# marbl/Mash

Measured on AMD Instinct MI355X. Metric: pairwise Mash distances/sec (s=1000), higher is better.
Workload: dtype u64; 1 GPU; mash triangle all-vs-all, 100000 clustered synthetic sketches, k=21 s=1000, 4999950000 pairs/step, per-table job (index build + discover + fill + merge each step), row-block sharded x1; parallelism=rowblock1, rccl_ranks=0

## Files before the change

### mash_amd/csrc/compare_dense.hip

```cpp
#ifdef MG_HIP_EMU
#include "hipemu.h"
#else
#include <hip/hip_runtime.h>
#define MG_DYN_SHARED(T, name)                                   \
    extern __shared__ __align__(16) unsigned char name##_raw[]; \
    T *name = reinterpret_cast<T *>(name##_raw)
#endif
#include <stdint.h>

#include <cstdlib>

#ifndef MG_HIP_EMU
#include <rocprim/device/device_radix_sort.hpp>
#include <rocprim/device/device_select.hpp>
#include <rocprim/iterator/counting_iterator.hpp>
#endif

#include "compare_internal.h"

namespace mg {

#ifndef MG_HIP_EMU
__global__ __launch_bounds__(256) void dn_neighbor_kernel(const uint64_t *hashes, uint64_t stride, const uint32_t *cnt, uint32_t n,
                                                          uint8_t *link)
// ... 299 lines not shown
            }
            nx += total;
            __syncthreads();
        }
    }
    __syncthreads();
    const uint32_t jb = (row - G.g0) >> 7, bl = (row - G.g0) & 127u;
    const uint64_t bw = dense_block_words(W);
    unsigned long long *blk = gdata + G.data_off + (uint64_t)jb * bw;
    uint16_t *cxp = reinterpret_cast<uint16_t *>(blk + 128ull * W), *totp = cxp + (W + 1u) * 128u;
    unsigned long long *xpl = blk + dense_block_planes(W);
    for (uint32_t i = tid; i < 16u * W; i += 256u) {
        const uint32_t four = gap8[i], w = i >> 4, q = i & 15u;
        uint32_t bits[4] = {0u, 0u, 0u, 0u}, over = 0;
#pragma unroll
        for (uint32_t e = 0; e < 4u; e++) {
            const uint32_t c = (four >> (8u * e)) & 255u;
            over |= c >= 16u ? 1u : 0u;
#pragma unroll
            for (uint32_t j = 0; j < 4u; j++) bits[j] |= ((c >> j) & 1u) << ((4u * q + e) & 31u);
        }
        if (over || (q == 0 && hist[w] >= 256u)) ovf[w] = 1u;
#pragma unroll
        for (uint32_t j = 0; j < 4u; j++)
            if (bits[j]) atomicOr(&pl32[2u * (4u * w + j) + (q >> 3)], bits[j]);
    }
    __syncthreads();
    for (uint32_t i = tid; i < 4u * W; i += 256u) xpl[i * 128u + bl] = (unsigned long long)pl32[2u * i] | ((unsigned long long)pl32[2u * i + 1u] << 32);
    if (tid == 0) {
        uint32_t run = 0, all = 0;
        for (uint32_t w = 0; w <= W; w++) {
            cxp[w * 128u + bl] = (uint16_t)(run | ((w > 0 && ovf[w - 1u]) ? DN_CX_FLAG : 0u));
            totp[w * 128u + bl] = (uint16_t)all;
            if (w < W) {
                run += hist[w];
                all += hist[w] + (uint32_t)__popc(mask32[2u * w]) + (uint32_t)__popc(mask32[2u * w + 1u]);
            }
        }
    }
    for (uint32_t w = tid; w < W; w += 256u)
        blk[w * 128u + bl] = (unsigned long long)mask32[2u * w] | ((unsigned long long)mask32[2u * w + 1u] << 32);
}

hipError_t launch_dense_encode(const uint32_t *off, const uint32_t *code_img, uint32_t *pos_img, uint32_t rs, const uint32_t *grp_of,
                               const DenseGroup *groups, const uint32_t *ulist, const uint32_t *upos, unsigned long long *gdata,
                               uint16_t *ext, uint32_t xs, uint32_t n, uint32_t wmax, hipStream_t stream, int ul_mode)
{
    if (n == 0) return hipSuccess;
    const size_t fixed = ((size_t)28 * wmax + 9) * 4, with_ul = fixed + (size_t)wmax * 64 * 4;
    const bool ul_in_lds = ul_mode == 0 ? false : ul_mode == 1 ? with_ul <= 150 * 1024 : with_ul <= 40 * 1024;
    const size_t smem = ul_in_lds ? with_ul : fixed;
    auto go = [&](auto kern) -> hipError_t {
        hipError_t e = hipFuncSetAttribute(reinterpret_cast<const void *>(kern), hipFuncAttributeMaxDynamicSharedMemorySize, (int)smem);
        if (e != hipSuccess) return e;
        hipLaunchKernelGGL(kern, dim3((n + 63u) & ~63u), dim3(256), smem, stream, off, code_img, pos_img, rs, grp_of, groups, ulist, upos, gdata, wmax, ext, xs,
                           n, ul_in_lds ? 1u : 0u);
        return hipGetLastError();
    };
    return rs >= 4096u ? go(dn_encode_kernel<8>) : go(dn_encode_kernel<1>);
}



__device__ __forceinline__ uint32_t dn_count_add(uint32_t x, uint32_t acc)
{
#ifdef MG_HIP_EMU
    return (uint32_t)__popc(x) + acc;
#else
    uint32_t d;
    asm("v_bcnt_u32_b32 %0, %1, %2" : "=v"(d) : "v"(x), "v"(acc));
    return d;
#endif
}

__device__ __forceinline__ uint32_t dn_low_bits(uint32_t x, uint32_t y)
{
#ifdef MG_HIP_EMU
    return x & ((1u << y) - 1u);
#else
    return __builtin_amdgcn_ubfe(x, 0u, y);
#endif
}

template <uint32_t NP>
__device__ __forceinline__ uint32_t dn_descend(uint32_t base, uint32_t s, uint32_t u1, uint32_t A0, uint32_t B0, uint32_t A1, uint32_t B1,
                                               uint32_t A2, uint32_t B2, uint32_t A3, uint32_t B3)
{
    uint32_t pos = 0;
#pragma unroll
    for (uint32_t bit = 16u; bit != 0u; bit >>= 1) {
        const uint32_t y = pos + bit;
        uint32_t c = dn_count_add(dn_low_bits(B0, y), dn_count_add(dn_low_bits(A0, y), dn_count_add(dn_low_bits(u1, y), base)));
        if (NP >= 1u) c += 2u * dn_count_add(dn_low_bits(B1, y), (uint32_t)__popc(dn_low_bits(A1, y)));
        if (NP >= 3u)
            c += 4u * dn_count_add(dn_low_bits(B2, y), (uint32_t)__popc(dn_low_bits(A2, y))) +
                 8u * dn_count_add(dn_low_bits(B3, y), (uint32_t)__popc(dn_low_bits(A3, y)));
        pos = c < s ? y : pos;
    }
    return pos;
}

__device__ __forceinline__ uint32_t dn_resolve(unsigned long long un, unsigned long long mab, uint32_t fprev, uint32_t s, uint32_t w, bool lists,
                                               const unsigned long long *xpa, const unsigned long long *xpb, const uint16_t *xa,
                                               const uint16_t *xb, uint32_t ca0, uint32_t na, uint32_t cb0, uint32_t nb)
{
    if (__ballot(lists) == 0) {
        const unsigned long long a0 = xpa[512u * w], a1 = xpa[512u * w + 128u], a2 = xpa[512u * w + 256u], a3 = xpa[512u * w + 384u];
        const unsigned long long b0 = xpb[512u * w], b1 = xpb[512u * w + 128u], b2 = xpb[512u * w + 256u], b3 = xpb[512u * w + 384u];
        const bool p1 = __ballot((a1 | b1) != 0ull) != 0, p23 = __ballot((a2 | a3 | b2 | b3) != 0ull) != 0;
        const uint32_t ulo = (uint32_t)un, uhi = (uint32_t)(un >> 32);
        uint32_t c31 = dn_count_add((uint32_t)b0, dn_count_add((uint32_t)a0, dn_count_add(ulo & 0x7FFFFFFFu, fprev)));
        if (p1 || p23) c31 += 2u * dn_count_add((uint32_t)b1, (uint32_t)__popc((uint32_t)a1));
        if (p23)
            c31 += 4u * dn_count_add((uint32_t)b2, (uint32_t)__popc((uint32_t)a2)) + 8u * dn_count_add((uint32_t)b3, (uint32_t)__popc((uint32_t)a3));
        const bool upper = c31 < s;
        const uint32_t base = upper ? c31 + (ulo >> 31) : fprev;
        const uint32_t u1 = (upper ? uhi : ulo) << 1;
        const uint32_t A0 = upper ? (uint32_t)(a0 >> 32) : (uint32_t)a0, B0 = upper ? (uint32_t)(b0 >> 32) : (uint32_t)b0;
        uint32_t pos;
        if (!p1 && !p23) {
            pos = dn_descend<0>(base, s, u1, A0, B0, 0, 0, 0, 0, 0, 0);
        } else {
            const uint32_t A1 = upper ? (uint32_t)(a1 >> 32) : (uint32_t)a1, B1 = upper ? (uint32_t)(b1 >> 32) : (uint32_t)b1;
            if (!p23) {
                pos = dn_descend<1>(base, s, u1, A0, B0, A1, B1, 0, 0, 0, 0);
            } else {
                const uint32_t A2 = upper ? (uint32_t)(a2 >> 32) : (uint32_t)a2, B2 = upper ? (uint32_t)(b2 >> 32) : (uint32_t)b2;
                const uint32_t A3 = upper ? (uint32_t)(a3 >> 32) : (uint32_t)a3, B3 = upper ? (uint32_t)(b3 >> 32) : (uint32_t)b3;
                pos = dn_descend<3>(base, s, u1, A0, B0, A1, B1, A2, B2, A3, B3);
            }
        }
        const uint32_t mlo = (uint32_t)mab, mhi = (uint32_t)(mab >> 32);
        return upper ? dn_count_add(dn_low_bits(mhi, pos), (uint32_t)__popc(mlo)) : (uint32_t)__popc(dn_low_bits(mlo, pos));
    }
    uint32_t lo = 0, hi = 63;
    const uint32_t wbase = w << 6;
    while (lo < hi) {
        const uint32_t mid = (lo + hi) >> 1;
        uint32_t c = fprev + (uint32_t)__popcll(un & ((1ull << mid) - 1ull));
        for (uint32_t k = 0; k < na; k++) c += ((uint32_t)xa[ca0 + k] - wbase <= mid) ? 1u : 0u;
        for (uint32_t k = 0; k < nb; k++) c += ((uint32_t)xb[cb0 + k] - wbase <= mid) ? 1u : 0u;
        if (c >= s) hi = mid; else lo = mid + 1u;
    }
    return (uint32_t)__popcll(mab & ((1ull << lo) - 1ull));
}

template <uint32_t DN_ROWS, uint32_t DN_IL>
__global__ __launch_bounds__(128) void dn_pairs_kernel(const DenseTile *tiles, const DenseGroup *groups, const unsigned long long *gdata,
                                                       uint32_t use_lists,
                                                       const uint16_t *ext, uint32_t xs, uint32_t s, uint32_t row_begin, uint32_t row_end,
                                                       uint64_t out_base, const uint32_t *inv, uint2 *out, DenseList list)
{
    MG_DYN_SHARED(unsigned long long, dl);
    const DenseTile T = tiles[blockIdx.x];
    const DenseGroup G = groups[T.group];
    const uint32_t W = G.W, tid = threadIdx.x;
    const uint64_t bw = dense_block_words(W);
    const unsigned long long *Bm = gdata + G.data_off + (uint64_t)T.cblk * bw;
    const uint16_t *Bcx = reinterpret_cast<const uint16_t *>(Bm + 128ull * W);
    const uint16_t *Btot = Bcx + (W + 1u) * 128u;
    unsigned long long *Am = dl;
    uint16_t *Acx = reinterpret_cast<uint16_t *>(Am + (uint64_t)DN_ROWS * W);
    uint16_t *Atot = Acx + (W + 1u) * DN_ROWS;
    const uint32_t ra = T.row0 - G.g0;
    const unsigned long long *asrc = gdata + G.data_off + (uint64_t)(ra >> 7) * bw;
    const uint32_t la0 = ra & 127u;
    for (uint32_t i = tid; i < W * DN_ROWS; i += 128u) Am[i] = asrc[(i / DN_ROWS) * 128u + la0 + (i % DN_ROWS)];
    {
        const uint16_t *acs = reinterpret_cast<const uint16_t *>(asrc + 128ull * W);
        for (uint32_t i = tid; i < 2u * (W + 1u) * DN_ROWS; i += 128u) Acx[i] = acs[(i / DN_ROWS) * 128u + la0 + (i % DN_ROWS)];
    }
    __syncthreads();
    constexpr uint32_t DN_NB = DN_ROWS / DN_IL;
    uint16_t *Amax = Atot + (W + 1u) * DN_ROWS;
    for (uint32_t i = tid; i < DN_NB * (W + 1u); i += 128u) {
        const uint32_t bt = i / (W + 1u), w = i - bt * (W + 1u);
        uint32_t m = 0;
        for (uint32_t k = 0; k < DN_IL; k++)
            if (T.row0 + bt * DN_IL + k < G.g1) {
                const uint32_t v = Atot[w * DN_ROWS + bt * DN_IL + k];
                m = v > m ? v : m;
            }
        Amax[i] = (uint16_t)m;
    }
    __syncthreads();
    const uint32_t b = G.g0 + T.cblk * 128u + tid;
    const uint32_t lb = b < G.g1 ? tid : G.g1 - 1u - (G.g0 + T.cblk * 128u);
    const uint16_t *xb = ext + (uint64_t)(G.xrow0 + (b < G.g1 ? b - G.g0 : 0u)) * xs;
    const unsigned long long *xpb = Bm + dense_block_planes(W) + lb;
    const uint32_t colrow = inv ? inv[G.g0 + T.cblk * 128u + lb] : G.g0 + T.cblk * 128u + lb;
    const uint64_t tri_col = (colrow ? (uint64_t)colrow * (colrow - 1u) / 2u : 0ull) - out_base;
    for (uint32_t ai = 0; ai < DN_ROWS; ai += DN_IL) {
        if (T.row0 + ai >= G.g1 || T.row0 + ai >= row_end) break;
        const uint16_t *amax = Amax + (ai / DN_IL) * (W + 1u);
        uint32_t common[DN_IL], nle[DN_IL];
#pragma unroll
        for (uint32_t k = 0; k < DN_IL; k++) common[k] = nle[k] = 0;
        unsigned long long mb_next = Bm[lb];
        uint32_t tb_next = Btot[128u + lb];
        uint32_t wi = 0;
        for (; wi < W; wi++) {
            if (__ballot((uint32_t)amax[wi + 1u] + tb_next > s) != 0) break;
            const unsigned long long mb = mb_next;
            if (wi + 1u < W) {
                mb_next = Bm[(wi + 1u) * 128u + lb];
                tb_next = Btot[(wi + 2u) * 128u + lb];
            }
            const uint32_t mlo = (uint32_t)mb, mhi = (uint32_t)(mb >> 32);
#pragma unroll
            for (uint32_t k = 0; k < DN_IL; k++) {
                const unsigned long long am = Am[wi * DN_ROWS + ai + k];
                common[k] = dn_count_add((uint32_t)am & mlo, dn_count_add((uint32_t)(am >> 32) & mhi, common[k]));
            }
        }
        const uint32_t nfast = wi;
        for (; wi < W; wi++) {
            const unsigned long long mb = mb_next;
            const int32_t tbs = (int32_t)tb_next - (int32_t)s;
            if (wi + 1u < W) {
                mb_next = Bm[(wi + 1u) * 128u + lb];
                tb_next = Btot[(wi + 2u) * 128u + lb];
            }
            const uint32_t mlo = (uint32_t)mb, mhi = (uint32_t)(mb >> 32);
            bool any = false;
#pragma unroll
            for (uint32_t k = 0; k < DN_IL; k++) {
                const unsigned long long am = Am[wi * DN_ROWS + ai + k];
                const uint32_t cnew = dn_count_add((uint32_t)am & mlo, dn_count_add((uint32_t)(am >> 32) & mhi, common[k]));
                const bool before = (int32_t)Atot[(wi + 1u) * DN_ROWS + ai + k] + tbs <= (int32_t)cnew;
                common[k] = before ? cnew : common[k];
                nle[k] += before ? 1u : 0u;
                any = any || before;
            }
            if (__ballot(any) == 0) break;
        }
#pragma unroll
        for (uint32_t k = 0; k < DN_IL; k++) {
            const uint32_t a = T.row0 + ai + k;
            const bool present = a < G.g1 && a < row_end && a >= row_begin && G.g0 + T.cblk * 128u < a;
            if (!present) continue;
            const bool valid = b < a;
            uint32_t denom = s;
            const uint32_t w = nfast + nle[k];
            const bool need = valid && w < W;
            if (__ballot(need) != 0) {
                const uint32_t wc = need ? w : 0u;
                const unsigned long long ma = Am[wc * DN_ROWS + ai + k], mb = Bm[wc * 128u + lb];
                const uint32_t ca0 = Acx[wc * DN_ROWS + ai + k] & DN_CX_MASK, ca1r = Acx[(wc + 1u) * DN_ROWS + ai + k];
                const uint32_t cb0 = Bcx[wc * 128u + lb] & DN_CX_MASK, cb1r = Bcx[(wc + 1u) * 128u + lb];
                const uint32_t fprev = (uint32_t)Atot[wc * DN_ROWS + ai + k] + (uint32_t)Btot[wc * 128u + lb] - common[k];
                const bool lists = need && (use_lists || ((ca1r | cb1r) & DN_CX_FLAG) != 0);
                const uint32_t add = dn_resolve(ma | mb, ma & mb, fprev, s, wc, lists, asrc + dense_block_planes(W) + la0 + ai + k, xpb,
                                               ext + (uint64_t)(G.xrow0 + (a - G.g0)) * xs, xb, ca0, need ? (ca1r & DN_CX_MASK) - ca0 : 0u, cb0,
                                               need ? (cb1r & DN_CX_MASK) - cb0 : 0u);
                if (need) common[k] += add;
            }
            if (!valid) continue;
            if (w >= W) {
                const uint32_t total = (uint32_t)Atot[W * DN_ROWS + ai + k] + (uint32_t)Btot[W * 128u + lb] - common[k];
                denom = total < s ? total : s;
            }
            if (list.rc) {
                const uint32_t ra = a - list.row_first;
                const uint32_t at = list.row_base[ra] + list.row_cnt[ra] - (a - b);
                list.rc[at] = make_uint2(a, b);
                list.counts[at] = make_uint2(common[k], denom);
            } else {
                const uint32_t arow = inv ? inv[a] : a;
                const uint64_t tri_a = (uint64_t)arow * (arow - 1u) / 2u - out_base;
                out[arow > colrow ? tri_a + colrow : tri_col + arow] = make_uint2(common[k], denom);
            }
        }
    }
}

uint32_t dense_max_words() { return 400; }

size_t dense_pairs_lds(uint32_t W, uint32_t rows) { return (size_t)rows * W * 8 + (size_t)(W + 1u) * rows * 4 + (size_t)(W + 1u) * 8 * 2 + 16; }

uint32_t dense_rows_per_tile(uint64_t wave_rows) { return wave_rows / 32u >= 16384u ? 32u : 8u; }

hipError_t launch_dense_pairs(const DenseTile *tiles, uint32_t ntiles, uint32_t rows_per_tile, const DenseGroup *groups,
                              const unsigned long long *gdata, bool use_lists, const uint16_t *ext, uint32_t xs,
                              uint32_t s, uint32_t wmax, uint32_t row_begin, uint32_t row_end, uint64_t out_base, const uint32_t *inv, uint2 *out,
                              hipStream_t stream, const DenseList *list)
{
    if (ntiles == 0) return hipSuccess;
    const size_t smem = dense_pairs_lds(wmax, rows_per_tile);
    auto go = [&](auto kern) -> hipError_t {
        hipError_t e = hipFuncSetAttribute(reinterpret_cast<const void *>(kern), hipFuncAttributeMaxDynamicSharedMemorySize, (int)smem);
        if (e != hipSuccess) return e;
        hipLaunchKernelGGL(kern, dim3(ntiles), dim3(128), smem, stream, tiles, groups, gdata, use_lists ? 1u : 0u, ext, xs, s, row_begin, row_end,
                           out_base, inv, out, list ? *list : DenseList());
        return hipGetLastError();
    };
    const uint32_t il = 8;
    if (rows_per_tile == 32u) return il >= 16u ? go(dn_pairs_kernel<32, 16>) : il >= 8u ? go(dn_pairs_kernel<32, 8>) : go(dn_pairs_kernel<32, 4>);
    return il >= 8u ? go(dn_pairs_kernel<8, 8>) : go(dn_pairs_kernel<8, 4>);
}

#ifndef MG_HIP_EMU
constexpr uint32_t CL_FIRST = 4;

__global__ __launch_bounds__(256) void cl_emit_kernel(const uint64_t *hashes, uint64_t stride, const uint32_t *cnt, uint32_t n,
                                                      unsigned long long *key, uint32_t *row_out, uint32_t *label)
{
    const uint32_t i = blockIdx.x * 256u + threadIdx.x;
    if (i >= n * CL_FIRST) return;
    const uint32_t row = i / CL_FIRST, f = i % CL_FIRST;
    key[i] = f < cnt[row] ? (unsigned long long)hashes[(uint64_t)row * stride + f] : ~0ull;
    row_out[i] = row;
    if (f == 0) label[row] = row;
}

__global__ __launch_bounds__(256) void cl_minrow_kernel(const unsigned long long *key_sorted, const uint32_t *row_sorted, uint32_t m,
                                                        uint32_t *label)
{
    const uint32_t i = blockIdx.x * 256u + threadIdx.x;
    if (i >= m) return;
    const unsigned long long k = key_sorted[i];
    if (k == ~0ull) return;
    uint32_t lo = 0, hi = i;
    while (lo < hi) {
        const uint32_t mid = (lo + hi) >> 1;
        if (key_sorted[mid] < k) lo = mid + 1; else hi = mid;
    }
    atomicMin(&label[row_sorted[i]], row_sorted[lo]);
}

__global__ __launch_bounds__(256) void cl_jump_kernel(const uint32_t *in, uint32_t *out, uint32_t n)
{
    const uint32_t i = blockIdx.x * 256u + threadIdx.x;
    if (i < n) out[i] = in[in[i]];
}

__global__ __launch_bounds__(256) void cl_order_keys_kernel(const uint32_t *label, uint32_t n, uint32_t split, unsigned long long *key)
{
    const uint32_t i = blockIdx.x * 256u + threadIdx.x;
    if (i < n) key[i] = ((unsigned long long)(i >= split ? 1u : 0u) << 63) | ((unsigned long long)label[i] << 32) | i;
}

__global__ __launch_bounds__(256) void cl_split_keys_kernel(const unsigned long long *key_sorted, uint32_t n, uint32_t *inv, uint32_t *label_sorted)
{
    const uint32_t i = blockIdx.x * 256u + threadIdx.x;
    if (i < n) {
        inv[i] = (uint32_t)(key_sorted[i] & 0xFFFFFFFFull);
        label_sorted[i] = (uint32_t)(key_sorted[i] >> 32) & 0x7FFFFFFFu;
    }
}

size_t dense_cluster_temp_bytes(uint32_t n)
{
    size_t a = 0, b = 0;
    rocprim::radix_sort_pairs(nullptr, a, (const unsigned long long *)nullptr, (unsigned long long *)nullptr, (const uint32_t *)nullptr,
                              (uint32_t *)nullptr, (size_t)n * CL_FIRST, 0u, 64u, (hipStream_t) nullptr);
    rocprim::radix_sort_keys(nullptr, b, (const unsigned long long *)nullptr, (unsigned long long *)nullptr, (size_t)n, 0u, 64u,
                             (hipStream_t) nullptr);
    return a > b ? a : b;
}

hipError_t dense_cluster_rows(const uint64_t *hashes, uint64_t stride, const uint32_t *cnt, uint32_t n, void *temp, size_t temp_bytes,
                              unsigned long long *key_a, unsigned long long *key_b, uint32_t *row_a, uint32_t *row_b, uint32_t *lab_a,
                              uint32_t *lab_b, uint32_t *inv, uint32_t *label_sorted, hipStream_t stream, uint32_t split)
{
    if (n == 0) return hipSuccess;
    const uint32_t m = n * CL_FIRST;
    hipLaunchKernelGGL(cl_emit_kernel, dim3((m + 255u) / 256u), dim3(256), 0, stream, hashes, stride, cnt, n, key_a, row_a, lab_a);
    hipError_t e = hipGetLastError();
    if (e != hipSuccess) return e;
    e = rocprim::radix_sort_pairs(temp, temp_bytes, (const unsigned long long *)key_a, key_b, (const uint32_t *)row_a, row_b, (size_t)m, 0u, 64u,
                                  stream);
    if (e != hipSuccess) return e;
    hipLaunchKernelGGL(cl_minrow_kernel, dim3((m + 255u) / 256u), dim3(256), 0, stream, (const unsigned long long *)key_b, (const uint32_t *)row_b, m,
                       lab_a);
    hipLaunchKernelGGL(cl_jump_kernel, dim3((n + 255u) / 256u), dim3(256), 0, stream, (const uint32_t *)lab_a, lab_b, n);
    hipLaunchKernelGGL(cl_jump_kernel, dim3((n + 255u) / 256u), dim3(256), 0, stream, (const uint32_t *)lab_b, lab_a, n);
    hipLaunchKernelGGL(cl_order_keys_kernel, dim3((n + 255u) / 256u), dim3(256), 0, stream, (const uint32_t *)lab_a, n, split, key_a);
    e = hipGetLastError();
    if (e != hipSuccess) return e;
    e = rocprim::radix_sort_keys(temp, temp_bytes, (const unsigned long long *)key_a, key_b, (size_t)n, 0u, 64u, stream);
    if (e != hipSuccess) return e;
    hipLaunchKernelGGL(cl_split_keys_kernel, dim3((n + 255u) / 256u), dim3(256), 0, stream, (const unsigned long long *)key_b, n, inv, label_sorted);
    return hipGetLastError();
}

__global__ __launch_bounds__(256) void cl_gather_rows_kernel(const uint64_t *hashes, uint64_t stride, const uint32_t *inv, uint64_t *out)
{
    const uint32_t a = blockIdx.x;
    const uint64_t *src = hashes + (uint64_t)inv[a] * stride;
    uint64_t *dst = out + (uint64_t)a * stride;
    for (uint64_t p = threadIdx.x; p < stride; p += 256u) dst[p] = src[p];
}

hipError_t launch_dense_gather_rows(const uint64_t *hashes, uint64_t stride, const uint32_t *inv, uint32_t n, uint64_t *out, hipStream_t stream)
{
    if (n == 0) return hipSuccess;
    hipLaunchKernelGGL(cl_gather_rows_kernel, dim3(n), dim3(256), 0, stream, hashes, stride, inv, out);
    return hipGetLastError();
}

#endif

__global__ __launch_bounds__(256) void dn_group_rows_kernel(const DenseGroup *groups, uint32_t ng, uint32_t n, uint32_t *grp_of, uint4 *lead_rows)
{
    const uint32_t r = blockIdx.x * 256u + threadIdx.x;
    if (r >= n) return;
    uint32_t lo = 0, hi = ng;
    while (lo < hi) {
        const uint32_t mid = (lo + hi) >> 1;
        if (groups[mid].g0 <= r) lo = mid + 1u;
        else hi = mid;
    }
    uint32_t g = 0xFFFFFFFFu, g0 = 0, g1 = 0;
    if (lo > 0 && r < groups[lo - 1u].g1) {
        g = lo - 1u;
        g0 = groups[g].g0;
        g1 = groups[g].g1;
    }
    grp_of[r] = g;
    lead_rows[r] = make_uint4(g, g0, g1, 0u);
}

hipError_t launch_dense_group_rows(const DenseGroup *groups, uint32_t ng, uint32_t n, uint32_t *grp_of, uint32_t *lead_rows, hipStream_t stream)
{
    if (n == 0) return hipSuccess;
    hipLaunchKernelGGL(dn_group_rows_kernel, dim3((n + 255u) / 256u), dim3(256), 0, stream, groups, ng, n, grp_of, reinterpret_cast<uint4 *>(lead_rows));
    return hipGetLastError();
}

}
```

### mash_amd/csrc/compare_internal.h

```cpp
#pragma once
#ifdef MG_HIP_EMU
#include "hipemu.h"
#else
#include <hip/hip_runtime.h>
#endif
#include <stdint.h>

namespace mg {

struct MergedTile {
    uint32_t rows[32];
    uint32_t col0, col1;
};

struct CompareArgs {
    const uint64_t *row_hashes;
    const uint32_t *row_nhash;
    const uint64_t *col_hashes;
    const uint32_t *col_nhash;
    const uint32_t *row_pfx;
    const uint32_t *col_pfx;
    const MergedTile *mtiles;
    uint2 *out;
    uint64_t row_stride, col_stride;
    uint64_t row_pfx_stride, col_pfx_stride;
    uint64_t row_begin, row_end;
    uint64_t ncols;
    uint64_t out_base;
    uint32_t s;
    uint32_t rows_per_tile;
    uint32_t triangle;
    uint32_t unroll;
    uint32_t pfx_shr;
    uint32_t nbuckets;
    unsigned long long *dbg;
    const uint32_t *row_win;
    const uint32_t *col_win;
    uint32_t win, nwin;
    uint32_t win_lo, win_hi;
    uint32_t win_ecap;
    uint8_t *win_mask;
    uint32_t win_kmax;
    uint32_t xcd_remap;
    uint32_t stage_pack;
};

bool compare_merged_supported(uint32_t s);
uint32_t compare_merged_rows(uint32_t s);
hipError_t launch_compare_merged(const CompareArgs &a, uint32_t ntiles, hipStream_t stream);
uint32_t compare_window_rows(uint32_t s);
uint32_t compare_window_entries();
uint32_t compare_window_row_entries();
hipError_t launch_window_offsets(const uint32_t *pfx, uint64_t pfx_stride, const uint32_t *nhash, uint64_t n, uint32_t s,
                                 uint32_t nwin, uint32_t delta, uint32_t *out, hipStream_t stream);
hipError_t launch_table_max(const uint64_t *hashes, const uint32_t *nhash, uint64_t n, uint64_t stride,
                            unsigned long long *out_max, hipStream_t stream);
hipError_t launch_row_classes(const uint64_t *hashes, const uint32_t *nhash, uint64_t n, uint64_t stride,
                              uint8_t *out, unsigned long long *last_out, hipStream_t stream);
uint64_t compare_pfx_stride(uint64_t s);
hipError_t launch_make_prefix(const uint64_t *hashes, const uint32_t *nhash, uint64_t n, uint64_t s,
                              uint64_t pfx_stride, uint32_t shr, uint32_t *out, hipStream_t stream);
hipError_t launch_compare_generic(const CompareArgs &a, hipStream_t stream);

struct DenseGroup;
struct SparseArgs {
    const uint32_t *sorted_rows;
    const uint32_t *lo_img;
    const uint32_t *hi_img;
    uint32_t lo_shift;
    const uint32_t *off;
    const uint32_t *row_img;
    const uint32_t *col_img;
    const uint32_t *col_cnt_off;
    uint32_t rs_row, rs_col;
    uint32_t row_begin, row_end;
    uint32_t ncols;
    uint32_t triangle;
    uint32_t s;
    uint64_t out_base;
    uint2 *cand;
    uint64_t cand_cap;
    unsigned long long *counters;
    uint2 *out;
    uint2 *res;
    unsigned long long *seg_base;
    uint32_t *seg_cnt;
    uint32_t *chunk_inc;
    const uint32_t *rep;
    const uint32_t *cls_of;
    const uint32_t *cls_off;
    const uint32_t *cls_rows;
    const uint32_t *gend;
    const uint32_t *order;
    const uint32_t *inv;
    const uint32_t *dn_grp_of;
    const DenseGroup *dn_groups;
};
size_t sparse_dup_temp_bytes(uint32_t n);
hipError_t launch_sparse_dup_suspects(const unsigned long long *dig, const uint32_t *cnt, uint32_t n, void *temp, size_t temp_bytes,
                                      unsigned long long *dig_sorted, uint32_t *rows_sorted, uint32_t *flags, uint32_t *nflag,
                                      hipStream_t stream);
size_t sparse_order_temp_bytes(uint32_t n);
hipError_t launch_sparse_row_order(const uint32_t *off, const uint32_t *code_img, const uint32_t *gend, const uint32_t *rep, uint32_t n,
                                   uint32_t rs, void *temp, size_t temp_bytes, unsigned long long *key_a, unsigned long long *key_b,
                                   uint32_t *order, hipStream_t stream);
size_t sparse_order_slice_temp_bytes(uint32_t n);
hipError_t launch_sparse_order_slice(const uint32_t *order, uint32_t n, uint32_t rb, uint32_t re, void *temp, size_t temp_bytes,
                                     uint32_t *out, uint32_t *count_out, hipStream_t stream);
hipError_t launch_sparse_class_pairs(uint2 *out, const uint32_t *cls_rows, const uint32_t *cls_first, const uint32_t *off,
                                     const uint32_t *rep, uint32_t members, uint32_t row_begin, uint32_t row_end, uint64_t out_base,
                                     const uint32_t *inv, hipStream_t stream);
hipError_t launch_sparse_row_digest(const uint64_t *hashes, uint64_t stride, const uint32_t *cnt, uint32_t n,
                                    unsigned long long *digest, hipStream_t stream);
hipError_t launch_sparse_row_equal(const uint64_t *hashes, uint64_t stride, const uint32_t *cnt, const uint2 *pairs, uint32_t npairs,
                                   uint32_t *equal, hipStream_t stream);
hipError_t launch_sparse_row_counts(const uint32_t *nhash, uint32_t n, uint32_t cap, uint32_t *cnt, hipStream_t stream);
size_t sparse_offsets_temp_bytes(uint32_t n);
hipError_t launch_sparse_offsets(const uint32_t *cnt, const uint32_t *inv, uint32_t n, void *temp, uint32_t *off, hipStream_t stream);
size_t sparse_sort_temp_bytes(uint32_t E, uint32_t end_bit, uint32_t begin_bit);
uint32_t sparse_img_stride(uint32_t s);
hipError_t sparse_build_index(const uint64_t *hashes, uint64_t stride, const uint32_t *off, uint32_t n, uint32_t E,
                              uint32_t rs, uint32_t end_bit, void *temp, size_t temp_bytes, uint64_t *keys_a,
                              uint32_t *idx_a, uint64_t *keys_sorted, uint32_t *idx_sorted, uint32_t *head, uint32_t *gs_of,
                              uint32_t *sorted_rows, uint32_t *gend, uint32_t *code_img, uint32_t *pos_img, void *stat_scratch,
                              uint32_t begin_bit, void *tie_scratch, unsigned long long *incidences, uint32_t *max_group, uint32_t *groups,
                              uint32_t *bad, uint32_t *tie_overflow, hipStream_t stream);
size_t sparse_stat_scratch_bytes();
uint32_t sparse_sort_begin_bit(uint32_t E, uint32_t end_bit, const char *forced_bits, bool all_bits);
size_t sparse_tie_scratch_bytes();
hipError_t launch_sparse_locate(const uint64_t *qhashes, uint64_t qstride, const uint32_t *qoff, uint32_t q_begin, uint32_t nq,
                                const uint64_t *keys_sorted, const uint32_t *gend, uint32_t E, uint32_t rs, uint32_t *qlo_img,
                                uint32_t *qhi_img, uint32_t *qcode_img, hipStream_t stream);
bool sparse_discover_supported(uint32_t ncols_max);
hipError_t launch_sparse_discover(const SparseArgs &a, bool count_only, hipStream_t stream);
hipError_t launch_sparse_merge(const SparseArgs &a, uint64_t expect, uint32_t cus, hipStream_t stream);
bool sparse_merge_rows_supported(uint32_t rs_row);
size_t sparse_scan_temp_bytes(uint32_t nrows);
hipError_t launch_sparse_merge_rows(const SparseArgs &a, uint64_t expect, uint32_t *chunks, void *temp, size_t temp_bytes,
                                    hipStream_t stream);
hipError_t launch_sparse_scatter(const SparseArgs &a, uint64_t expect, uint32_t cus, hipStream_t stream);
size_t sparse_gather_temp_bytes(uint32_t nrows);
hipError_t launch_sparse_gather_rows(const SparseArgs &a, uint32_t *cnt_by_row, uint32_t *row_base, void *temp, size_t temp_bytes, uint32_t row_add,
                                     uint2 *rc_out, uint2 *counts_out, hipStream_t stream);
size_t sparse_edges_temp_bytes(uint64_t K);
uint64_t sparse_edges_blocks(uint64_t K);
hipError_t launch_sparse_list_edges(const uint2 *rc, const uint2 *counts, uint64_t K, uint32_t *blk_cnt, uint32_t *blk_off, void *temp, size_t temp_bytes,
                                    uint4 *edges, unsigned long long *total, hipStream_t stream);
uint64_t sparse_fill_chunks(uint64_t pairs);
constexpr uint32_t kFillStop = 0x80000000u;
hipError_t launch_sparse_fill_chunks(uint2 *out, uint64_t pairs, uint32_t numer, uint32_t denom, uint32_t blocks, uint32_t naps, uint32_t *ctr,
                                     hipStream_t stream, uint32_t threads = 256);
hipError_t launch_sparse_fill_value(uint2 *out, uint64_t pairs, uint32_t numer, uint32_t denom, uint32_t blocks_per_cu, uint32_t cus,
                                    hipStream_t stream);
hipError_t launch_sparse_merge_pack(const SparseArgs &a, uint64_t expect, uint32_t *chunks, void *temp, size_t temp_bytes, bool *used,
                                    hipStream_t stream);
hipError_t launch_sparse_fill_short(uint2 *out, const uint32_t *short_rows, const uint32_t *short_rcnt, uint32_t nshort_rows,
                                    const uint32_t *short_cols, const uint32_t *short_ccnt, uint32_t nshort_cols,
                                    uint32_t row_begin, uint32_t ncols, uint32_t triangle, uint64_t out_base, uint32_t s,
                                    const uint32_t *inv, hipStream_t stream);

struct DenseGroup {
    uint32_t g0, g1;
    uint32_t ustart, u;
    uint32_t W;
    uint32_t xrow0;
    uint64_t data_off;
};
struct DenseTile { uint32_t group, row0, cblk; };
#ifdef __HIPCC__
__host__ __device__
#endif
static inline uint64_t dense_block_planes(uint32_t W) { return 128ull * W + 64ull * (W + 1u); }
#ifdef __HIPCC__
__host__ __device__
#endif
static inline uint64_t dense_block_words(uint32_t W) { return dense_block_planes(W) + 512ull * W; }
struct DenseList {
    const uint32_t *row_base = nullptr, *row_cnt = nullptr;
    uint2 *rc = nullptr, *counts = nullptr;
    uint32_t row_first = 0;
};
hipError_t launch_dense_neighbors(const uint64_t *hashes, uint64_t stride, const uint32_t *cnt, uint32_t n, uint8_t *link,
                                  hipStream_t stream);
size_t dense_universe_temp_bytes(uint32_t cap);
uint32_t dense_sublists();
hipError_t dense_find_leaders(const uint32_t *sorted_rows, const uint32_t *gs_of, const uint32_t *gend, const uint32_t *grp_of,
                              const DenseGroup *groups, uint32_t E, unsigned long long *key, uint32_t *val, uint32_t cap_sub,
                              unsigned long long *key_out, uint32_t *val_out, uint32_t *cnt, uint32_t *off, uint32_t *total,
                              hipStream_t stream);
hipError_t dense_join_leaders(const unsigned long long *key, const uint32_t *val, uint32_t cap_sub, unsigned long long *key_out, uint32_t *val_out,
                              const uint32_t *cnt, uint32_t *off, uint32_t *total, hipStream_t stream);
hipError_t dense_sort_universes(const unsigned long long *key, const uint32_t *val, uint32_t m, void *temp, size_t temp_bytes,
                                unsigned long long *key_sorted, uint32_t *ulist, uint32_t *upos, uint32_t *ustart, uint32_t *uend,
                                uint32_t group_bits, hipStream_t stream);
hipError_t launch_dense_encode(const uint32_t *off, const uint32_t *code_img, uint32_t *pos_img, uint32_t rs, const uint32_t *grp_of,
                               const DenseGroup *groups, const uint32_t *ulist, const uint32_t *upos, unsigned long long *gdata,
                               uint16_t *ext, uint32_t xs, uint32_t n, uint32_t wmax, hipStream_t stream, int ul_mode = -1);
size_t dense_pairs_lds(uint32_t W, uint32_t rows);
uint32_t dense_rows_per_tile(uint64_t wave_rows);
uint32_t dense_max_words();
hipError_t launch_dense_pairs(const DenseTile *tiles, uint32_t ntiles, uint32_t rows_per_tile, const DenseGroup *groups,
                              const unsigned long long *gdata, bool use_lists, const uint16_t *ext, uint32_t xs,
                              uint32_t s, uint32_t wmax, uint32_t row_begin, uint32_t row_end, uint64_t out_base, const uint32_t *inv, uint2 *out,
                              hipStream_t stream, const DenseList *list = nullptr);
size_t dense_cluster_temp_bytes(uint32_t n);
hipError_t dense_cluster_rows(const uint64_t *hashes, uint64_t stride, const uint32_t *cnt, uint32_t n, void *temp, size_t temp_bytes,
                              unsigned long long *key_a, unsigned long long *key_b, uint32_t *row_a, uint32_t *row_b, uint32_t *lab_a,
                              uint32_t *lab_b, uint32_t *inv, uint32_t *label_sorted, hipStream_t stream, uint32_t split = 0);
hipError_t launch_dense_gather_rows(const uint64_t *hashes, uint64_t stride, const uint32_t *inv, uint32_t n, uint64_t *out, hipStream_t stream);
hipError_t launch_dense_group_rows(const DenseGroup *groups, uint32_t ng, uint32_t n, uint32_t *grp_of, uint32_t *lead_rows, hipStream_t stream);

struct JoinSide {
    const uint2 *grp = nullptr;
    const uint32_t *ent = nullptr;
    const uint32_t *goff = nullptr;
    const uint32_t *gend = nullptr;
    const uint32_t *thr = nullptr;
};
struct JoinArgs {
    JoinSide rows, cols;
    const uint32_t *row_cnt_off, *col_cnt_off;
    const uint32_t *rep, *col_rep;
    const uint32_t *inv;
    uint2 *out;
    uint64_t out_base;
    uint64_t ntiles;
    uint32_t ncols;
    uint32_t row_begin, row_end;
    uint32_t bi0;
    uint32_t ncb;
    uint32_t triangle, s;
    uint32_t tiles_per_wg = 1;
};
size_t join_order_temp_bytes(uint32_t nrows);
hipError_t join_order_rows(const uint32_t *img, uint32_t rs, const uint32_t *cnt_off, const uint32_t *rep, const uint32_t *inv, const uint32_t *gend,
                           const uint32_t *sorted_rows, uint32_t nrows, void *temp, size_t temp_bytes, uint32_t *lab, unsigned long long *key_a,
                           unsigned long long *key_b, uint32_t *val_a, uint32_t *perm, uint32_t *src, uint32_t *map, hipStream_t stream, uint32_t split = 0);
uint32_t join_block_rows();
uint32_t join_levels();
size_t join_build_temp_bytes(uint64_t slots);
hipError_t join_build_lists(const uint32_t *img, uint32_t rs, const uint32_t *cnt_off, const uint32_t *rep, uint32_t nrows, uint32_t s, uint32_t E,
                            bool only_shared, void *temp, size_t temp_bytes, unsigned long long *key_a, unsigned long long *key_b, uint32_t *val_a,
                            uint32_t *val_b, uint2 *grp, uint32_t *goff, uint32_t *gend, uint32_t *thr, const uint32_t **ent_out, hipStream_t stream);
hipError_t launch_join_levels(const uint32_t *img, uint32_t rs, const uint32_t *cnt_off, const uint32_t *rep, uint32_t nrows, uint32_t s,
                              uint32_t *thr, hipStream_t stream);
hipError_t launch_join_shared(const uint32_t *lo_img, const uint32_t *hi_img, uint32_t lo_shift, uint32_t rs, const uint32_t *cnt_off,
                              uint32_t row_begin, uint32_t row_end, unsigned long long *sum, hipStream_t stream);
hipError_t launch_join_tiles(const JoinArgs &a, hipStream_t stream);

struct FilterArgs {
    const uint2 *counts;
    const uint32_t *min_numer;
    uint32_t *seg_count;
    unsigned long long *seg_off;
    uint4 *edges;
    uint64_t pairs;
    uint64_t first_row;
    uint64_t ncols;
    uint64_t win_lo, win_n;
    uint32_t s;
    uint32_t triangle;
};
uint64_t filter_segments(uint64_t pairs);
hipError_t launch_filter_count(const FilterArgs &a, unsigned long long *total, hipStream_t stream);
hipError_t launch_filter_write(const FilterArgs &a, hipStream_t stream);

}
```

### mash_amd/csrc/compare_sparse.hip

```cpp
#include <hip/hip_runtime.h>
#include <stdint.h>

#include <cstdlib>
#include <cstring>
#include <rocprim/device/device_radix_sort.hpp>
#include <rocprim/device/device_scan.hpp>
#include <rocprim/device/device_select.hpp>
#include <rocprim/iterator/counting_iterator.hpp>

#include "compare_internal.h"

namespace mg {


__global__ __launch_bounds__(256) void sp_fill_entries_kernel(const uint64_t *hashes, uint64_t stride, const uint32_t *off,
                                                              uint32_t rs, uint64_t *keys, uint32_t *idx)
{
    const uint32_t row = blockIdx.x;
    const uint32_t b = off[row], cnt = off[row + 1] - b;
    const uint64_t *src = hashes + (uint64_t)row * stride;
    const uint32_t ib = row * rs;
    for (uint32_t p = threadIdx.x; p < cnt; p += 256) {
        keys[b + p] = src[p];
        idx[b + p] = ib + p;
    }
}

__global__ __launch_bounds__(256) void sp_heads_kernel(const uint64_t *keys, const uint32_t *idx, uint32_t E, uint32_t *head,
                                                       uint32_t *bad)
{
    const uint32_t pos = blockIdx.x * 256u + threadIdx.x;
    if (pos >= E) return;
    uint32_t h = pos;
    if (pos > 0) {
        const uint64_t k = keys[pos], kp = keys[pos - 1];
        if (k == kp) {
            h = 0;
            if (idx[pos] <= idx[pos - 1]) *bad = 1;
        } else if (k < kp) {
            *bad = 1;
        }
    }
    head[pos] = h;
}

constexpr uint32_t SP_STAT_SLOTS = 1024;
struct SpStatSlot { unsigned long long inc; uint32_t max_group, groups; };

__global__ __launch_bounds__(256) void sp_index_scatter_kernel(const uint32_t *idx, const uint32_t *gs_of, uint32_t E,
                                                               uint32_t rs, uint32_t *sorted_rows, uint32_t *gend, uint32_t *code_img,
                                                               uint32_t *pos_img, SpStatSlot *stat)
{
    const uint32_t pos = blockIdx.x * 256u + threadIdx.x;
    unsigned long long inc = 0;
    uint32_t glen = 0, heads = 0;
    if (pos < E) {
        const uint32_t i = idx[pos];
        const uint32_t gs = gs_of[pos];
        const bool last = pos + 1u == E || gs_of[pos + 1u] != gs;
        const bool shared = !(last && gs == pos);
        sorted_rows[pos] = i / rs;
        code_img[i] = (gs << 1) | (shared ? 1u : 0u);
        pos_img[i] = pos;
        inc = pos - gs;
        heads = gs == pos ? 1u : 0u;
        if (last) {
            gend[gs] = pos + 1u;
            glen = pos + 1u - gs;
        }
    }
    for (int d = 32; d > 0; d >>= 1) {
        inc += __shfl_xor(inc, d);
        heads += __shfl_xor(heads, d);
        const uint32_t o = __shfl_xor(glen, d);
        glen = o > glen ? o : glen;
    }
    __shared__ unsigned long long s_inc[4];
    __shared__ uint32_t s_len[4], s_heads[4];
    if ((threadIdx.x & 63) == 0) { s_inc[threadIdx.x >> 6] = inc; s_len[threadIdx.x >> 6] = glen; s_heads[threadIdx.x >> 6] = heads; }
    __syncthreads();
    if (threadIdx.x == 0) {
        SpStatSlot *sl = stat + (blockIdx.x & (SP_STAT_SLOTS - 1u));
        const unsigned long long t = s_inc[0] + s_inc[1] + s_inc[2] + s_inc[3];
        uint32_t m = s_len[0];
        for (int w = 1; w < 4; w++) m = s_len[w] > m ? s_len[w] : m;
        if (t) atomicAdd(&sl->inc, t);
        if (m > 1) atomicMax(&sl->max_group, m);
        atomicAdd(&sl->groups, s_heads[0] + s_heads[1] + s_heads[2] + s_heads[3]);
    }
}

__global__ __launch_bounds__(256) void sp_stat_reduce_kernel(const SpStatSlot *stat, unsigned long long *incidences, uint32_t *max_group,
                                                             uint32_t *groups)
{
    unsigned long long inc = 0;
    uint32_t m = 0, g = 0;
    for (uint32_t i = threadIdx.x; i < SP_STAT_SLOTS; i += 256u) {
        inc += stat[i].inc;
        m = stat[i].max_group > m ? stat[i].max_group : m;
        g += stat[i].groups;
    }
    if (inc) atomicAdd(incidences, inc);
    if (m) atomicMax(max_group, m);
    if (g) atomicAdd(groups, g);
}

size_t sparse_stat_scratch_bytes() { return sizeof(SpStatSlot) * SP_STAT_SLOTS; }

__global__ __launch_bounds__(256) void sp_entry_counts_kernel(const uint32_t *nhash, uint32_t n, uint32_t cap, uint32_t *cnt)
{
    const uint32_t i = blockIdx.x * 256u + threadIdx.x;
    if (i < n) cnt[i] = nhash[i] < cap ? nhash[i] : cap;
}

hipError_t launch_sparse_row_counts(const uint32_t *nhash, uint32_t n, uint32_t cap, uint32_t *cnt, hipStream_t stream)
{
    if (n == 0) return hipSuccess;
    hipLaunchKernelGGL(sp_entry_counts_kernel, dim3((n + 255u) / 256u), dim3(256), 0, stream, nhash, n, cap, cnt);
    return hipGetLastError();
}

__global__ __launch_bounds__(1024) void sp_offsets_sums_kernel(const uint32_t *cnt, const uint32_t *inv, uint32_t n, uint32_t *part)
{
    __shared__ uint32_t s_part[16];
    const uint32_t tid = threadIdx.x, a = blockIdx.x * 1024u + tid;
    uint32_t c = a < n ? cnt[inv ? inv[a] : a] : 0u;
#pragma unroll
    for (uint32_t d = 32; d > 0; d >>= 1) c += __shfl_xor(c, d);
    if ((tid & 63u) == 0) s_part[tid >> 6] = c;
    __syncthreads();
    if (tid == 0) {
        uint32_t t = 0;
        for (uint32_t k = 0; k < 16u; k++) t += s_part[k];
        part[blockIdx.x] = t;
    }
}

__global__ __launch_bounds__(1024) void sp_offsets_scan_kernel(const uint32_t *cnt, const uint32_t *inv, uint32_t n, const uint32_t *part, uint32_t *off)
{
    __shared__ uint32_t s_part[16], s_base[16];
    const uint32_t tid = threadIdx.x, lane = tid & 63u, wid = tid >> 6, a = blockIdx.x * 1024u + tid;
    uint32_t before = 0;
    for (uint32_t k = tid; k < blockIdx.x; k += 1024u) before += part[k];
#pragma unroll
    for (uint32_t d = 32; d > 0; d >>= 1) before += __shfl_xor(before, d);
    if (lane == 0) s_base[wid] = before;
    const uint32_t c = a < n ? cnt[inv ? inv[a] : a] : 0u;
    uint32_t incl = c;
#pragma unroll
    for (uint32_t d = 1; d < 64u; d <<= 1) {
        const uint32_t y = __shfl_up(incl, d);
        if (lane >= d) incl += y;
    }
    if (lane == 63u) s_part[wid] = incl;
    __syncthreads();
    uint32_t run = incl - c;
    for (uint32_t k = 0; k < 16u; k++) run += s_base[k] + (k < wid ? s_part[k] : 0u);
    if (a < n) off[a] = run;
    if (a + 1u == n) off[n] = run + c;
}

size_t sparse_offsets_temp_bytes(uint32_t n) { return ((size_t)n / 1024u + 1u) * 4u; }

hipError_t launch_sparse_offsets(const uint32_t *cnt, const uint32_t *inv, uint32_t n, void *temp, uint32_t *off, hipStream_t stream)
{
    if (n == 0) return hipMemsetAsync(off, 0, 4, stream);
    const uint32_t nb = (n + 1023u) / 1024u;
    hipLaunchKernelGGL(sp_offsets_sums_kernel, dim3(nb), dim3(1024), 0, stream, cnt, inv, n, static_cast<uint32_t *>(temp));
    hipLaunchKernelGGL(sp_offsets_scan_kernel, dim3(nb), dim3(1024), 0, stream, cnt, inv, n, static_cast<const uint32_t *>(temp), off);
    return hipGetLastError();
}

__global__ __launch_bounds__(256) void sp_fill_u32_kernel(uint32_t *p, uint64_t count, uint32_t v)
{
    const uint64_t stride = (uint64_t)gridDim.x * 256u;
    for (uint64_t i = (uint64_t)blockIdx.x * 256u + threadIdx.x; i < count; i += stride) p[i] = v;
}


__global__ __launch_bounds__(256) void sp_row_digest_kernel(const uint64_t *hashes, uint64_t stride, const uint32_t *cnt,
                                                            unsigned long long *digest)
{
    const uint32_t row = blockIdx.x;
    const uint32_t n = cnt[row];
    const uint64_t *src = hashes + (uint64_t)row * stride;
    unsigned long long h = 0;
    for (uint32_t p = threadIdx.x; p < n; p += 256) {
        unsigned long long z = src[p] + 0x9E3779B97F4A7C15ull * (unsigned long long)(p + 1);
        z = (z ^ (z >> 30)) * 0xBF58476D1CE4E5B9ull;
        z = (z ^ (z >> 27)) * 0x94D049BB133111EBull;
        h += z ^ (z >> 31);
    }
    for (int d = 32; d > 0; d >>= 1) h += __shfl_xor(h, d);
    __shared__ unsigned long long s_h[4];
    if ((threadIdx.x & 63) == 0) s_h[threadIdx.x >> 6] = h;
    __syncthreads();
    if (threadIdx.x == 0) digest[row] = s_h[0] + s_h[1] + s_h[2] + s_h[3];
}

__global__ __launch_bounds__(256) void sp_row_equal_kernel(const uint64_t *hashes, uint64_t stride, const uint32_t *cnt,
                                                           const uint2 *pairs, uint32_t npairs, uint32_t *equal)
{
    const uint32_t k = blockIdx.x;
    if (k >= npairs) return;
    const uint2 pr = pairs[k];
    const uint32_t n = cnt[pr.x];
    int diff = cnt[pr.y] != n;
    const uint64_t *x = hashes + (uint64_t)pr.x * stride, *y = hashes + (uint64_t)pr.y * stride;
    for (uint32_t p = threadIdx.x; p < n && !diff; p += 256) diff |= x[p] != y[p];
    diff = __syncthreads_or(diff);
    if (threadIdx.x == 0) equal[k] = diff ? 0u : 1u;
}

hipError_t launch_sparse_row_digest(const uint64_t *hashes, uint64_t stride, const uint32_t *cnt, uint32_t n,
                                    unsigned long long *digest, hipStream_t stream)
{
    if (n == 0) return hipSuccess;
    hipLaunchKernelGGL(sp_row_digest_kernel, dim3(n), dim3(256), 0, stream, hashes, stride, cnt, digest);
    return hipGetLastError();
}

hipError_t launch_sparse_row_equal(const uint64_t *hashes, uint64_t stride, const uint32_t *cnt, const uint2 *pairs, uint32_t npairs,
                                   uint32_t *equal, hipStream_t stream)
{
    if (npairs == 0) return hipSuccess;
    hipLaunchKernelGGL(sp_row_equal_kernel, dim3(npairs), dim3(256), 0, stream, hashes, stride, cnt, pairs, npairs, equal);
    return hipGetLastError();
}

__global__ __launch_bounds__(256) void sp_dup_flags_kernel(const unsigned long long *dig_sorted, const uint32_t *rows_sorted,
                                                           const uint32_t *cnt, uint32_t n, uint32_t *flags, uint32_t *nflag)
{
    const uint32_t k = blockIdx.x * 256u + threadIdx.x;
    if (k >= n) return;
    uint32_t f = 0;
    if (k > 0 && dig_sorted[k] == dig_sorted[k - 1]) {
        const uint32_t c = cnt[rows_sorted[k]];
        f = (c != 0 && c == cnt[rows_sorted[k - 1]]) ? 1u : 0u;
    }
    flags[k] = f;
    if (f) atomicAdd(nflag, 1u);
}

size_t sparse_dup_temp_bytes(uint32_t n)
{
    size_t b = 0;
    rocprim::radix_sort_pairs(nullptr, b, (const unsigned long long *)nullptr, (unsigned long long *)nullptr,
                              rocprim::counting_iterator<uint32_t>(0u), (uint32_t *)nullptr, (size_t)n, 0u, 64u, (hipStream_t) nullptr);
    return b;
}

hipError_t launch_sparse_dup_suspects(const unsigned long long *dig, const uint32_t *cnt, uint32_t n, void *temp, size_t temp_bytes,
                                      unsigned long long *dig_sorted, uint32_t *rows_sorted, uint32_t *flags, uint32_t *nflag,
                                      hipStream_t stream)
{
    if (n == 0) return hipSuccess;
    hipError_t e = hipMemsetAsync(nflag, 0, 4, stream);
    if (e != hipSuccess) return e;
    e = rocprim::radix_sort_pairs(temp, temp_bytes, dig, dig_sorted, rocprim::counting_iterator<uint32_t>(0u), rows_sorted, (size_t)n, 0u, 64u,
                                  stream);
    if (e != hipSuccess) return e;
    hipLaunchKernelGGL(sp_dup_flags_kernel, dim3((n + 255u) / 256u), dim3(256), 0, stream, dig_sorted, rows_sorted, cnt, n, flags, nflag);
    return hipGetLastError();
}

__global__ __launch_bounds__(256) void sp_row_key_kernel(const uint32_t *off, const uint32_t *code_img, const uint32_t *gend,
                                                         const uint32_t *rep, uint32_t n, uint32_t rs, unsigned long long *key64)
{
    const uint32_t row = blockIdx.x * 4u + (threadIdx.x >> 6), lane = threadIdx.x & 63u;
    if (row >= n) return;
    const uint32_t er = rep ? rep[row] : row;
    const uint32_t cnt = off[er + 1] - off[er];
    uint32_t k = 0xFFFFFFFFu;
    for (uint32_t base = 0; base < cnt; base += 64u) {
        const uint32_t p = base + lane;
        const uint32_t code = p < cnt ? code_img[(uint64_t)er * rs + p] : 0u;
        const uint64_t m = __ballot((code & 1u) != 0);
        if (m != 0) {
            k = (uint32_t)__builtin_amdgcn_readlane((int)code, __builtin_ctzll(m)) >> 1;
            break;
        }
    }
    if (lane == 0) key64[row] = ((unsigned long long)k << 32) | (unsigned long long)(0xFFFFFFFFu - row);
}

__global__ __launch_bounds__(256) void sp_order_from_keys_kernel(const unsigned long long *key64_sorted, uint32_t n, uint32_t *order)
{
    const uint32_t i = blockIdx.x * 256u + threadIdx.x;
    if (i < n) order[i] = 0xFFFFFFFFu - (uint32_t)(key64_sorted[i] & 0xFFFFFFFFull);
}

size_t sparse_order_temp_bytes(uint32_t n)
{
    size_t b = 0;
    rocprim::radix_sort_keys(nullptr, b, (const unsigned long long *)nullptr, (unsigned long long *)nullptr, (size_t)n, 0u, 64u,
                             (hipStream_t) nullptr);
    return b;
}

hipError_t launch_sparse_row_order(const uint32_t *off, const uint32_t *code_img, const uint32_t *gend, const uint32_t *rep, uint32_t n,
                                   uint32_t rs, void *temp, size_t temp_bytes, unsigned long long *key_a, unsigned long long *key_b,
                                   uint32_t *order, hipStream_t stream)
{
    if (n == 0) return hipSuccess;
    hipLaunchKernelGGL(sp_row_key_kernel, dim3((n + 3u) / 4u), dim3(256), 0, stream, off, code_img, gend, rep, n, rs, key_a);
    hipError_t e = hipGetLastError();
    if (e != hipSuccess) return e;
    e = rocprim::radix_sort_keys(temp, temp_bytes, (const unsigned long long *)key_a, key_b, (size_t)n, 0u, 64u, stream);
    if (e != hipSuccess) return e;
    hipLaunchKernelGGL(sp_order_from_keys_kernel, dim3((n + 255u) / 256u), dim3(256), 0, stream, (const unsigned long long *)key_b, n, order);
    return hipGetLastError();
}

struct sp_in_range {
    uint32_t rb, re;
    __device__ bool operator()(const uint32_t &r) const { return r >= rb && r < re; }
};

size_t sparse_order_slice_temp_bytes(uint32_t n)
{
    size_t b = 0;
    rocprim::select(nullptr, b, (const uint32_t *)nullptr, (uint32_t *)nullptr, (uint32_t *)nullptr, (size_t)n, sp_in_range{0u, 0u},
                    (hipStream_t) nullptr);
    return b;
}

hipError_t launch_sparse_order_slice(const uint32_t *order, uint32_t n, uint32_t rb, uint32_t re, void *temp, size_t temp_bytes,
                                     uint32_t *out, uint32_t *count_out, hipStream_t stream)
{
    return rocprim::select(temp, temp_bytes, order, out, count_out, (size_t)n, sp_in_range{rb, re}, stream);
}

uint32_t sparse_img_stride(uint32_t s) { return ((s + 3u) & ~3u) + 4u; }

struct sp_max_u32 {
    __device__ uint32_t operator()(const uint32_t &a, const uint32_t &b) const { return a > b ? a : b; }
};

size_t sparse_sort_temp_bytes(uint32_t E, uint32_t end_bit, uint32_t begin_bit)
{
    size_t bytes = 0;
    rocprim::radix_sort_pairs(nullptr, bytes, (const uint64_t *)nullptr, (uint64_t *)nullptr, (const uint32_t *)nullptr,
                              (uint32_t *)nullptr, (size_t)E, 0u, end_bit, (hipStream_t) nullptr);
    size_t b1 = 0;
    rocprim::radix_sort_pairs(nullptr, b1, (const uint64_t *)nullptr, (uint64_t *)nullptr, (const uint32_t *)nullptr,
                              (uint32_t *)nullptr, (size_t)E, begin_bit, end_bit, (hipStream_t) nullptr);
    bytes = bytes > b1 ? bytes : b1;
    size_t b2 = 0;
    rocprim::inclusive_scan(nullptr, b2, (const uint32_t *)nullptr, (uint32_t *)nullptr, (size_t)E, sp_max_u32(), (hipStream_t) nullptr);
    return bytes > b2 ? bytes : b2;
}

constexpr uint32_t SP_TIE_WALK = 1024, SP_TIE_CAP = 1u << 16, SP_TIE_VALUES = 64;

__global__ __launch_bounds__(256) void sp_tie_find_kernel(const uint64_t *keys, uint32_t E, uint32_t bb, uint32_t *breaks, uint32_t *nbreak,
                                                          uint32_t *overflow)
{
    const uint32_t pos = blockIdx.x * 256u + threadIdx.x;
    if (pos == 0 || pos >= E) return;
    const uint64_t k = keys[pos], kp = keys[pos - 1];
    if ((kp >> bb) != (k >> bb) || k == kp) return;
    const uint32_t slot = atomicAdd(nbreak, 1u);
    if (slot >= SP_TIE_CAP) { *overflow = 1; return; }
    breaks[slot] = pos;
}

__global__ __launch_bounds__(64) void sp_tie_segments_kernel(const uint64_t *keys, uint32_t E, uint32_t bb, const uint32_t *breaks,
                                                             const uint32_t *nbreak, uint2 *segs, uint32_t *nseg, uint32_t *overflow)
{
    const uint32_t m = *nbreak < SP_TIE_CAP ? *nbreak : SP_TIE_CAP;
    if (blockIdx.x >= m) return;
    const uint32_t lane = threadIdx.x;
    const uint32_t pos = breaks[blockIdx.x];
    const uint64_t kp = keys[pos - 1];
    const uint64_t prefix = kp >> bb;
    uint32_t s0 = 0;
    {
        uint32_t hi = pos - 1;
        uint32_t chunks = 0;
        for (;;) {
            if (hi == 0) { s0 = 0; break; }
            const bool in = lane < hi;
            const uint64_t k = in ? keys[hi - 1u - lane] : 0;
            const bool other_prefix = in && (k >> bb) != prefix;
            const bool other_value = in && !other_prefix && k != kp;
            const uint64_t stop = __ballot(other_prefix || other_value);
            if (stop) {
                const uint32_t first = (uint32_t)__builtin_ctzll(stop);
                if ((__ballot(other_value) >> first) & 1ull) return;
                s0 = hi - first;
                break;
            }
            if (hi <= 64u) { s0 = 0; break; }
            hi -= 64u;
            if (++chunks > SP_TIE_WALK) { if (lane == 0) *overflow = 1; return; }
        }
    }
    uint32_t s1 = E;
    {
        uint32_t lo = pos;
        uint32_t chunks = 0;
        for (;;) {
            if (lo >= E) { s1 = E; break; }
            const uint32_t q = lo + lane;
            const bool out = q < E && (keys[q] >> bb) != prefix;
            const uint64_t stop = __ballot(out);
            if (stop) { s1 = lo + (uint32_t)__builtin_ctzll(stop); break; }
            lo += 64u;
            if (++chunks > SP_TIE_WALK) { if (lane == 0) *overflow = 1; return; }
        }
    }
    if (lane == 0) segs[atomicAdd(nseg, 1u)] = make_uint2(s0, s1);
}

__global__ __launch_bounds__(64) void sp_tie_repair_kernel(uint64_t *keys, uint32_t *idx, const uint2 *segs, const uint32_t *nseg, uint64_t *tk,
                                                           uint32_t *ti, uint32_t *overflow)
{
    if (blockIdx.x >= *nseg) return;
    const uint32_t lane = threadIdx.x;
    const uint32_t s0 = segs[blockIdx.x].x, s1 = segs[blockIdx.x].y;
    uint32_t out = s0, rounds = 0;
    bool have = false;
    uint64_t last = 0;
    while (out < s1) {
        uint64_t best = ~0ull;
        for (uint32_t q = s0 + lane; q < s1; q += 64u) {
            const uint64_t k = keys[q];
            if ((!have || k > last) && k < best) best = k;
        }
        for (uint32_t d = 32; d; d >>= 1) {
            const uint64_t o = __shfl_xor(best, d, 64);
            best = o < best ? o : best;
        }
        if (++rounds > SP_TIE_VALUES) { if (lane == 0) *overflow = 1; return; }
        for (uint32_t base = s0; base < s1; base += 64u) {
            const uint32_t q = base + lane;
            const bool hit = q < s1 && keys[q] == best;
            const uint64_t bal = __ballot(hit);
            if (hit) {
                const uint32_t w = out + (uint32_t)__popcll(bal & ((1ull << lane) - 1ull));
                tk[w] = best;
                ti[w] = idx[q];
            }
            out += (uint32_t)__popcll(bal);
        }
        last = best;
        have = true;
    }
    __threadfence();
    for (uint32_t q = s0 + lane; q < s1; q += 64u) {
        keys[q] = __hip_atomic_load(&tk[q], __ATOMIC_RELAXED, __HIP_MEMORY_SCOPE_AGENT);
        idx[q] = __hip_atomic_load(&ti[q], __ATOMIC_RELAXED, __HIP_MEMORY_SCOPE_AGENT);
    }
}

uint32_t sparse_sort_begin_bit(uint32_t E, uint32_t end_bit, const char *forced_bits, bool all_bits)
{
    if (all_bits || end_bit >= 64u) return 0;
    const char *forced = forced_bits;
    if (!forced && E < (1u << 22)) return 0;
    uint32_t lg = 0;
    while ((1ull << lg) < (uint64_t)E) lg++;
    const uint32_t want = 2u * lg > 29u ? 2u * lg - 13u : 16u;
    uint32_t passes = (want + 7u) / 8u;
    if (passes > 1u && want - (passes - 1u) * 8u <= 2u) passes--;
    uint32_t bits = passes * 8u;
    if (forced) bits = (uint32_t)atoi(forced);
    if (bits < 8u) bits = 8u;
    if (bits + 8u > end_bit) return 0;
    return end_bit - bits;
}

size_t sparse_tie_scratch_bytes() { return (size_t)SP_TIE_CAP * (sizeof(uint32_t) + sizeof(uint2)) + 16; }

hipError_t sparse_build_index(const uint64_t *hashes, uint64_t stride, const uint32_t *off, uint32_t n, uint32_t E,
                              uint32_t rs, uint32_t end_bit, void *temp, size_t temp_bytes, uint64_t *keys_a,
                              uint32_t *idx_a, uint64_t *keys_sorted, uint32_t *idx_sorted, uint32_t *head, uint32_t *gs_of,
                              uint32_t *sorted_rows, uint32_t *gend, uint32_t *code_img, uint32_t *pos_img, void *stat_scratch,
                              uint32_t begin_bit, void *tie_scratch, unsigned long long *incidences, uint32_t *max_group, uint32_t *groups,
                              uint32_t *bad, uint32_t *tie_overflow, hipStream_t stream)
{
    if (n == 0 || E == 0) return hipSuccess;
    hipLaunchKernelGGL(sp_fill_entries_kernel, dim3(n), dim3(256), 0, stream, hashes, stride, off, rs, keys_a, idx_a);
    hipError_t e = hipGetLastError();
    if (e != hipSuccess) return e;
    e = rocprim::radix_sort_pairs(temp, temp_bytes, (const uint64_t *)keys_a, keys_sorted, (const uint32_t *)idx_a, idx_sorted,
                                  (size_t)E, begin_bit, end_bit, stream);
    if (e != hipSuccess) return e;
    const uint32_t blocks = (E + 255u) / 256u;
    if (begin_bit > 0) {
        uint2 *segs = static_cast<uint2 *>(tie_scratch);
        uint32_t *breaks = reinterpret_cast<uint32_t *>(segs + SP_TIE_CAP);
        uint32_t *nbreak = breaks + SP_TIE_CAP, *nseg = nbreak + 1;
        e = hipMemsetAsync(nbreak, 0, 8, stream);
        if (e != hipSuccess) return e;
        hipLaunchKernelGGL(sp_tie_find_kernel, dim3(blocks), dim3(256), 0, stream, (const uint64_t *)keys_sorted, E, begin_bit, breaks, nbreak, tie_overflow);
        hipLaunchKernelGGL(sp_tie_segments_kernel, dim3(SP_TIE_CAP), dim3(64), 0, stream, (const uint64_t *)keys_sorted, E, begin_bit,
                           (const uint32_t *)breaks, (const uint32_t *)nbreak, segs, nseg, tie_overflow);
        hipLaunchKernelGGL(sp_tie_repair_kernel, dim3(SP_TIE_CAP), dim3(64), 0, stream, keys_sorted, idx_sorted, (const uint2 *)segs,
                           (const uint32_t *)nseg, keys_a, idx_a, tie_overflow);
        e = hipGetLastError();
        if (e != hipSuccess) return e;
    }
    hipLaunchKernelGGL(sp_heads_kernel, dim3(blocks), dim3(256), 0, stream, keys_sorted, idx_sorted, E, head, bad);
    e = hipGetLastError();
    if (e != hipSuccess) return e;
    e = rocprim::inclusive_scan(temp, temp_bytes, (const uint32_t *)head, gs_of, (size_t)E, sp_max_u32(), stream);
    if (e != hipSuccess) return e;
    {
        const uint64_t total = (uint64_t)n * rs;
        uint64_t fb = (total + 1023) / 1024;
        if (fb > 8192) fb = 8192;
        hipLaunchKernelGGL(sp_fill_u32_kernel, dim3((uint32_t)fb), dim3(256), 0, stream, code_img, total, 0xFFFFFFFFu);
        e = hipGetLastError();
        if (e != hipSuccess) return e;
    }
    e = hipMemsetAsync(stat_scratch, 0, sparse_stat_scratch_bytes(), stream);
    if (e != hipSuccess) return e;
    hipLaunchKernelGGL(sp_index_scatter_kernel, dim3(blocks), dim3(256), 0, stream, (const uint32_t *)idx_sorted, (const uint32_t *)gs_of, E, rs,
                       sorted_rows, gend, code_img, pos_img, static_cast<SpStatSlot *>(stat_scratch));
    e = hipGetLastError();
    if (e != hipSuccess) return e;
    hipLaunchKernelGGL(sp_stat_reduce_kernel, dim3(1), dim3(256), 0, stream, static_cast<const SpStatSlot *>(stat_scratch), incidences, max_group,
                       groups);
    return hipGetLastError();
}


__global__ __launch_bounds__(256) void sp_locate_kernel(const uint64_t *qhashes, uint64_t qstride, const uint32_t *qoff,
                                                        uint32_t q_begin, uint32_t nq, const uint64_t *keys_sorted,
                                                        const uint32_t *gend, uint32_t E, uint32_t rs, uint32_t *qlo_img,
                                                        uint32_t *qhi_img, uint32_t *qcode_img)
{
    const uint32_t q = blockIdx.x;
    if (q >= nq) return;
    const uint32_t cnt = qoff[q + 1] - qoff[q];
    const uint64_t *src = qhashes + (uint64_t)(q_begin + q) * qstride;
    for (uint32_t p = threadIdx.x; p < cnt; p += 256) {
        const uint64_t v = src[p];
        uint32_t lo = 0, hi = E;
        while (lo < hi) {
            const uint32_t mid = lo + ((hi - lo) >> 1);
            if (keys_sorted[mid] < v) lo = mid + 1; else hi = mid;
        }
        const bool found = lo < E && keys_sorted[lo] == v;
        const uint64_t at = (uint64_t)q * rs + p;
        qcode_img[at] = found ? (lo << 1) + 1u : (lo << 1);
        qlo_img[at] = lo;
        qhi_img[at] = found ? gend[lo] : lo;
    }
}


__device__ __forceinline__ uint32_t sp_class_span(const SparseArgs &a, uint32_t c, uint32_t row, uint32_t &first)
{
    const uint32_t k = a.cls_of[c];
    if (k == 0xFFFFFFFFu) { first = 0xFFFFFFFFu; return 1u; }
    const uint32_t lo = a.cls_off[k], hi = a.cls_off[k + 1];
    first = lo;
    if (!a.triangle) return hi - lo;
    uint32_t l = lo, h = hi;
    while (l < h) {
        const uint32_t mid = (l + h) >> 1;
        if (a.cls_rows[mid] < row) l = mid + 1; else h = mid;
    }
    return l - lo;
}

template <bool COUNT_ONLY, bool DEDUP>
__global__ __launch_bounds__(256) void sp_discover_kernel(SparseArgs a)
{
    extern __shared__ uint32_t bm[];
    __shared__ uint32_t s_w[4];
    __shared__ unsigned long long s_base;
    __shared__ unsigned long long s_inc[4];
    const uint32_t row = a.order ? a.order[blockIdx.x] : a.row_end - 1u - blockIdx.x;
    const uint32_t tid = threadIdx.x, lane = tid & 63u, wid = tid >> 6;
    const uint32_t ncols = a.triangle ? row : a.ncols;
    const uint32_t W = (ncols + 31u) >> 5;
    const uint32_t er = (DEDUP && a.triangle) ? a.rep[row] : row;
    const bool copy = DEDUP && a.triangle && er != row;
    const uint32_t cnt = a.off[er + 1] - a.off[er];
    if (cnt == 0 || ncols == 0) return;
    if (!copy) {
        int any = 0;
        for (uint32_t p = tid; p < cnt; p += 256u) {
            const uint64_t at = (uint64_t)er * a.rs_row + p;
            any |= (a.lo_img[at] >> a.lo_shift) != a.hi_img[at];
        }
        if (__syncthreads_or(any) == 0) return;
    }
    for (uint32_t w = tid; w < W; w += 256) bm[w] = 0;
    __syncthreads();
    unsigned long long inc = 0;
    constexpr uint32_t SHORT = 6;
    for (uint32_t base = wid * 64u; base < cnt; base += 256u) {
        const uint32_t p = base + lane;
        uint2 lh = make_uint2(0u, 0u);
        if (p < cnt) {
            const uint64_t at = (uint64_t)er * a.rs_row + p;
            lh = make_uint2(a.lo_img[at] >> a.lo_shift, a.hi_img[at]);
            if (copy) lh.y = a.gend[lh.x];
        }
        const uint32_t len = lh.y - lh.x;
        inc += len;
        if (len != 0 && len <= SHORT) {
            for (uint32_t t = 0; t < len; t++) {
                const uint32_t r = a.sorted_rows[lh.x + t];
                if (copy && r >= row) break;
                if (copy && r == er) continue;
                if (!((bm[r >> 5] >> (r & 31u)) & 1u)) atomicOr(&bm[r >> 5], 1u << (r & 31u));
            }
        }
        auto mark = [&](uint32_t r) {
// ... 916 lines not shown
```

### mash_amd/csrc/host_index.cpp

```cpp
#include "host_internal.h"
#include "index_build.h"
#ifdef IX_PHASE_CLOCKS
namespace mg { void index_dump_clocks(); }
#endif
#include "sort_bits.h"

namespace {

const uint64_t kTilesLongestRun = 6144;
static const uint64_t kSplitMinRun = 128;

uint64_t longest_label_run(const uint32_t *lab_sorted, uint64_t n)
{
    if (!lab_sorted || n == 0) return 0;
    uint64_t run = 1, longest = 1;
    for (uint64_t a = 1; a < n; a++) {
        run = lab_sorted[a] == lab_sorted[a - 1] ? run + 1 : 1;
        longest = std::max(longest, run);
    }
    return longest;
}

struct SparseIndexBuild {
    mg_ctx *ctx;
    const mg_table *t;
    const uint32_t s;
    const bool clustered;
    const uint32_t split;
    mg_table::Sparse *sp;
    const uint64_t n;
    const std::chrono::steady_clock::time_point t_begin = std::chrono::steady_clock::now();
    bool stop = false;

    bool need_classes = false, dedup = true, want_dense = true, try_cluster = false, try_links = false;
    DevBuf<uint8_t> dc_cls, d_link;
    DevBuf<unsigned long long> dc_last, d_dig, d_dig_sorted, k_a, k_b;
    DevBuf<uint32_t> d_cnt, d_rows_sorted, d_flags, d_nflag, r_a, r_b, l_a, l_b, d_inv, d_lab;
    DevBuf<unsigned char> d_tmp_dup, d_tmp_cl;
    std::vector<uint8_t> hc_cls, link;
    std::vector<uint64_t> hc_last;
    std::vector<uint32_t> hc_nh, inv_v, lab_v;
    const uint32_t *inv = nullptr, *lab_sorted = nullptr;
    uint32_t nflag = 0;
    size_t tb_dup = 0, tb_cl = 0;
    bool cluster_q = false, links_q = false;

    const char *ix_mode = nullptr;
    bool ix_verify = false, ix_tiles = true;
    std::vector<uint32_t> cnt_true, cnt_perm;
    uint32_t max_cnt = 0;
    uint64_t maxv = 0, E_all = 0;
    double dens[65] = {0};
    double dens0 = 0;
    std::vector<uint32_t> rep;
    const uint64_t *H = nullptr;
    mg::IxPlan early_plan;
    DevBuf<unsigned char> d_lb;
    bool lb_made = false;
    bool cnt_stale = false;

    std::vector<uint32_t> cls_of, cls_off, cls_rows, cls_first;

    uint32_t E = 0, end_bit = 0, sort_begin_bit = 0;
    std::vector<mg::DenseGroup> cand_groups;
    std::vector<uint32_t> grp_of_h;
    DevBuf<mg::DenseGroup> d_groups;
    DevBuf<uint32_t> d_grp_of, d_lead_rows, d_val, d_valj, d_cnt_sub, d_off_sub, d_nlead;
    DevBuf<unsigned long long> d_key, d_keyj;
    uint32_t lead_lists = 0, lead_tot[2] = {0, 0}, lead_cap = 0;
    bool lead_ready = false, lead_done = false, cand_prepared = false;
    mg::IxPlan plan;
    size_t temp_bytes = 0;
    DevBuf<unsigned char> temp;
    DevBuf<uint32_t> gs_of;
    DevBuf<unsigned long long> key64_a, key64_b;
    struct Stat { unsigned long long shared; uint32_t max_group, groups, bad, tie_overflow; uint32_t ixf[4]; } h_stat = {0, 0, 0, 0, 0, {0, 0, 0, 0}};
    DevBuf<Stat> d_stat;
    DevBuf<unsigned char> d_slots;
    bool want_order = true, ok = false;
    size_t nshort = 0;
    std::vector<uint32_t> short_cnt;
    hipError_t e = hipSuccess;

    bool built = false;

    SparseIndexBuild(mg_ctx *c, const mg_table *tab, uint32_t sketch_size, bool clustered_variant, mg_table::Sparse *index, uint32_t split_row)
        : ctx(c), t(tab), s(sketch_size), clustered(clustered_variant), split(split_row), sp(index), n(tab->n), dc_cls(c), d_link(c), dc_last(c), d_dig(c),
          d_dig_sorted(c), k_a(c), k_b(c), d_cnt(c), d_rows_sorted(c), d_flags(c), d_nflag(c), r_a(c), r_b(c), l_a(c), l_b(c), d_inv(c),
          d_lab(c), d_tmp_dup(c), d_tmp_cl(c), d_lb(c), d_groups(c), d_grp_of(c), d_lead_rows(c), d_val(c), d_valj(c), d_cnt_sub(c),
          d_off_sub(c), d_nlead(c), d_key(c), d_keyj(c), temp(c), gs_of(c), key64_a(c), key64_b(c), d_stat(c), d_slots(c)
    {
    }

    int unusable(const char *why)
    {
        sp->usable = false;
        sp->why = why;
        stop = true;
        return MG_OK;
    }

    hipError_t counts_to_device()
    {
            if (!cnt_stale) return hipSuccess;
            cnt_stale = false;
            return hipMemcpyAsync(d_cnt, cnt_true.data(), n * 4, hipMemcpyHostToDevice, ctx->stream);
    }

    template <class T> bool take(T **p, size_t count)
    {
        void *q = nullptr;
        if (ctx_malloc(ctx, &q, std::max<size_t>(count, 1) * sizeof(T)) != hipSuccess) return false;
        *p = static_cast<T *>(q);
        return true;
    }

    void drop()
    {
            for (void **q : {(void **)&sp->off, (void **)&sp->keys_sorted, (void **)&sp->gend, (void **)&sp->sorted_rows, (void **)&sp->code_img,
                             (void **)&sp->pos_img, (void **)&sp->short_rows, (void **)&sp->short_cnt, (void **)&sp->counters, (void **)&sp->order,
                             (void **)&sp->rep, (void **)&sp->cls_of, (void **)&sp->cls_off, (void **)&sp->cls_rows, (void **)&sp->cls_first})
                if (*q) { ctx_free(ctx, *q); *q = nullptr; }
    }

    int scan_rows();
    int order_rows();
    int find_copies();
    int lay_out();
    void prepare_candidates();
    void finish_build();
    int build_by_tiles();
    int build_by_sort();
    int check_build();
    int dense_groups();
    int run();
};

int SparseIndexBuild::scan_rows()
{
    need_classes = t->cls.size() != n;
    dedup = !ctx_opt(ctx, "MASHGPU_SPARSE_NO_DEDUP");
    want_dense = true;
    if (const char *v = ctx_opt(ctx, "MASHGPU_COMPARE_DENSE")) want_dense = atoi(v) != 0;
    try_cluster = clustered && n >= 16;
    try_links = !try_cluster && want_dense && n >= 8 && s <= 16384;
    tb_dup = mg::sparse_dup_temp_bytes((uint32_t)n);
    tb_cl = mg::dense_cluster_temp_bytes((uint32_t)n);
    if (d_cnt.alloc(n) != hipSuccess || (need_classes && (dc_cls.alloc(n) != hipSuccess || dc_last.alloc(n) != hipSuccess)) ||
        (dedup && (d_dig.alloc(n) != hipSuccess || d_dig_sorted.alloc(n) != hipSuccess || d_rows_sorted.alloc(n) != hipSuccess ||
                   d_flags.alloc(n) != hipSuccess || d_nflag.alloc(1) != hipSuccess || d_tmp_dup.alloc(std::max<size_t>(tb_dup, 16)) != hipSuccess))) {
        (void)hipGetLastError();
        return unusable("no device memory for the index");
    }
    {
        hipError_t e = hipSuccess;
        if (need_classes) {
            hc_cls.resize(n);
            hc_last.resize(n);
            hc_nh.resize(n);
            e = mg::launch_row_classes(t->hashes, t->nhash, n, t->s, dc_cls, dc_last, ctx->stream);
        }
        if (e == hipSuccess) e = mg::launch_sparse_row_counts(t->nhash, (uint32_t)n, (uint32_t)std::min<uint64_t>(t->s, s), d_cnt, ctx->stream);
        if (e == hipSuccess && dedup) {
            e = mg::launch_sparse_row_digest(t->hashes, t->s, d_cnt, (uint32_t)n, d_dig, ctx->stream);
            if (e == hipSuccess)
                e = mg::launch_sparse_dup_suspects(d_dig, d_cnt, (uint32_t)n, d_tmp_dup, tb_dup, d_dig_sorted, d_rows_sorted, d_flags, d_nflag, ctx->stream);
        }
        if (e == hipSuccess && try_cluster) {
            if (k_a.alloc(4 * n) == hipSuccess && k_b.alloc(4 * n) == hipSuccess && r_a.alloc(4 * n) == hipSuccess && r_b.alloc(4 * n) == hipSuccess &&
                l_a.alloc(n) == hipSuccess && l_b.alloc(n) == hipSuccess && d_inv.alloc(n) == hipSuccess && d_lab.alloc(n) == hipSuccess &&
                d_tmp_cl.alloc(std::max<size_t>(tb_cl, 16)) == hipSuccess) {
                e = mg::dense_cluster_rows(t->hashes, t->s, d_cnt, (uint32_t)n, d_tmp_cl, tb_cl, k_a, k_b, r_a, r_b, l_a, l_b, d_inv, d_lab, ctx->stream, split);
                cluster_q = true;
            } else {
                (void)hipGetLastError();
            }
        }
        if (e == hipSuccess && try_links) {
            if (d_link.alloc(n) == hipSuccess) {
                link.resize(n);
                e = mg::launch_dense_neighbors(t->hashes, t->s, d_cnt, (uint32_t)n, d_link, ctx->stream);
                links_q = true;
            } else {
                (void)hipGetLastError();
            }
        }
        const size_t pin_bytes = 8 * n + 4 * n + 4 * n + 4 * n + 8 + n + n + 64;
        unsigned char *pin = static_cast<unsigned char *>(ctx_pinned(ctx, pin_bytes));
        unsigned long long *p_last = pin ? reinterpret_cast<unsigned long long *>(pin) : nullptr;
        uint32_t *p_nh = pin ? reinterpret_cast<uint32_t *>(pin + 8 * n) : nullptr, *p_inv = pin ? p_nh + n : nullptr, *p_lab = pin ? p_inv + n : nullptr;
        uint32_t *p_nflag = pin ? p_lab + n : &nflag;
        uint8_t *p_cls = pin ? pin + 20 * n + 8 : nullptr, *p_link = pin ? p_cls + n : nullptr;
        if (!pin) {
            if (cluster_q) { inv_v.resize(n); lab_v.resize(n); p_inv = inv_v.data(); p_lab = lab_v.data(); }
            p_nh = hc_nh.data(); p_cls = hc_cls.data(); p_last = reinterpret_cast<unsigned long long *>(hc_last.data()); p_link = link.data();
        }
        if (e == hipSuccess && need_classes) {
            e = hipMemcpyAsync(p_nh, t->nhash, n * 4, hipMemcpyDeviceToHost, ctx->stream);
            if (e == hipSuccess) e = hipMemcpyAsync(p_cls, dc_cls, n, hipMemcpyDeviceToHost, ctx->stream);
            if (e == hipSuccess) e = hipMemcpyAsync(p_last, dc_last, n * 8, hipMemcpyDeviceToHost, ctx->stream);
        }
        if (e == hipSuccess && dedup) e = hipMemcpyAsync(p_nflag, d_nflag, 4, hipMemcpyDeviceToHost, ctx->stream);
        if (e == hipSuccess && cluster_q) {
            e = hipMemcpyAsync(p_inv, d_inv, n * 4, hipMemcpyDeviceToHost, ctx->stream);
            if (e == hipSuccess) e = hipMemcpyAsync(p_lab, d_lab, n * 4, hipMemcpyDeviceToHost, ctx->stream);
        }
        if (e == hipSuccess && links_q) e = hipMemcpyAsync(p_link, d_link, n, hipMemcpyDeviceToHost, ctx->stream);
        const hipError_t es = hipStreamSynchronize(ctx->stream);
        if (e == hipSuccess) e = es;
        if (e == hipSuccess && pin) {
            if (need_classes) {
                memcpy(hc_nh.data(), p_nh, n * 4);
                memcpy(hc_cls.data(), p_cls, n);
                memcpy(hc_last.data(), p_last, n * 8);
            }
            if (dedup) nflag = *p_nflag;
            if (links_q) memcpy(link.data(), p_link, n);
        }
        if (cluster_q) { inv = p_inv; lab_sorted = p_lab; }
        if (e != hipSuccess) return fail(ctx, MG_ERR_HIP, std::string("compare (index: rows, copies, order): ") + hipGetErrorString(e));
    }
    if (need_classes) {
        t->cls.swap(hc_cls);
        t->last.swap(hc_last);
        t->nh.swap(hc_nh);
    }
    if (!links_q) link.clear();
    return MG_OK;
}

int SparseIndexBuild::order_rows()
{
    ix_mode = ctx_opt(ctx, "MASHGPU_SPARSE_INDEX");
    ix_verify = ix_mode && strcmp(ix_mode, "verify") == 0;
    ix_tiles = !ix_mode || strcmp(ix_mode, "sort") != 0;
    cnt_true.assign(n, 0);
    for (uint64_t i = 0; i < n; i++) {
        const uint32_t c = (uint32_t)std::min<uint64_t>(std::min<uint64_t>(t->nh[i], t->s), s);
        cnt_true[i] = c;
        E_all += c;
        max_cnt = std::max(max_cnt, c);
        if (c) {
            const uint64_t last = t->last[i];
            if (last == MG_HASH_PAD) return unusable("a hash equals the padding value");
            maxv = std::max(maxv, last);
            const double d = (double)c / ((double)last + 1.0);
            dens[64 - __builtin_clzll(last | 1ull)] += d;
            dens0 += d;
        }
    }
    H = t->hashes;
    bool keep_table_order = false;
    if (cluster_q && split != 0 && lab_sorted && !ctx_opt(ctx, "MASHGPU_SPLIT_ALWAYS") && longest_label_run(lab_sorted, n) * (uint64_t)s < kSplitMinRun * 1000ull) {
        keep_table_order = true;
        lab_sorted = nullptr;
    }
    if (cluster_q) {
        bool identity = true;
        for (uint64_t a = 0; a < n && identity; a++) identity = inv[a] == a;
        if (!identity && !keep_table_order) {
            void *pi = nullptr, *ph = nullptr;
            if (ctx_malloc(ctx, &pi, n * 4) != hipSuccess || ctx_malloc(ctx, &ph, std::max<uint64_t>(n * t->s, 1) * 8) != hipSuccess) {
                (void)hipGetLastError();
                ctx_free(ctx, pi);
                lab_sorted = nullptr;
            } else {
                sp->inv = static_cast<uint32_t *>(pi);
                sp->phashes = static_cast<uint64_t *>(ph);
                HIP_TRY(ctx, hipMemcpyAsync(sp->inv, d_inv, n * 4, hipMemcpyDeviceToDevice, ctx->stream));
                if (ix_tiles && !(dedup && nflag) && E_all > 0 && E_all < (1ull << 31) && longest_label_run(lab_sorted, n) <= kTilesLongestRun) {
                    early_plan = mg::index_plan((uint32_t)n, (uint32_t)E_all, s, sp->rs, t->s, maxv, dens0, ix_verify);
                    if (early_plan.ok && d_lb.alloc(early_plan.lb_bytes) == hipSuccess) {
                        HIP_TRY(ctx, mg::index_gather_rows(early_plan, t->hashes, sp->inv, d_cnt, sp->phashes, d_lb, ctx->stream));
                        lb_made = true;
                    } else {
                        (void)hipGetLastError();
                    }
                }
                if (!lb_made) HIP_TRY(ctx, mg::launch_dense_gather_rows(t->hashes, t->s, sp->inv, (uint32_t)n, sp->phashes, ctx->stream));
                H = sp->phashes;
                cnt_perm.resize(n);
                for (uint64_t a = 0; a < n; a++) cnt_perm[a] = cnt_true[inv[a]];
                cnt_true.swap(cnt_perm);
                cnt_stale = true;
            }
        }
    } else {
        lab_sorted = nullptr;
    }
    if (want_dense && n >= 8 && s <= 16384 && lab_sorted) {
        link.assign(n, 0);
        for (uint64_t a = 1; a < n; a++) link[a] = (a != split && lab_sorted[a] == lab_sorted[a - 1] && cnt_true[a] && cnt_true[a - 1]) ? 1 : 0;
    } else if (cluster_q && want_dense && n >= 8 && s <= 16384 && d_link.alloc(n) == hipSuccess) {
        link.resize(n);
        HIP_TRY(ctx, counts_to_device());
        HIP_TRY(ctx, mg::launch_dense_neighbors(H, t->s, d_cnt, (uint32_t)n, d_link, ctx->stream));
        HIP_TRY(ctx, hipMemcpyAsync(link.data(), d_link, n, hipMemcpyDeviceToHost, ctx->stream));
        HIP_TRY(ctx, hipStreamSynchronize(ctx->stream));
    } else if (!links_q) {
        (void)hipGetLastError();
        link.clear();
    }
    return MG_OK;
}

int SparseIndexBuild::find_copies()
{
    if (dedup && nflag) {
        HIP_TRY(ctx, counts_to_device());
        HIP_TRY(ctx, mg::launch_sparse_row_digest(H, t->s, d_cnt, (uint32_t)n, d_dig, ctx->stream));
        HIP_TRY(ctx, mg::launch_sparse_dup_suspects(d_dig, d_cnt, (uint32_t)n, d_tmp_dup, tb_dup, d_dig_sorted, d_rows_sorted, d_flags, d_nflag, ctx->stream));
        HIP_TRY(ctx, hipMemcpyAsync(&nflag, d_nflag, 4, hipMemcpyDeviceToHost, ctx->stream));
        HIP_TRY(ctx, hipStreamSynchronize(ctx->stream));
        if (nflag) {
            std::vector<uint32_t> rows_sorted(n), flags(n);
            HIP_TRY(ctx, hipMemcpyAsync(rows_sorted.data(), d_rows_sorted, n * 4, hipMemcpyDeviceToHost, ctx->stream));
            HIP_TRY(ctx, hipMemcpyAsync(flags.data(), d_flags, n * 4, hipMemcpyDeviceToHost, ctx->stream));
            HIP_TRY(ctx, hipStreamSynchronize(ctx->stream));
            std::vector<uint2> pairs;
            pairs.reserve(nflag);
            for (uint64_t k = 1, g0 = 0; k < n; k++) {
                if (flags[k]) pairs.push_back(make_uint2(rows_sorted[k], rows_sorted[g0]));
                else g0 = k;
            }
            DevBuf<uint2> d_pairs(ctx);
            DevBuf<uint32_t> d_eq(ctx);
            if (d_pairs.alloc(pairs.size()) != hipSuccess || d_eq.alloc(pairs.size()) != hipSuccess) { (void)hipGetLastError(); return unusable("no device memory for the index"); }
            std::vector<uint32_t> eq(pairs.size());
            HIP_TRY(ctx, hipMemcpyAsync(d_pairs, pairs.data(), pairs.size() * sizeof(uint2), hipMemcpyHostToDevice, ctx->stream));
            HIP_TRY(ctx, mg::launch_sparse_row_equal(H, t->s, d_cnt, d_pairs, (uint32_t)pairs.size(), d_eq, ctx->stream));
            HIP_TRY(ctx, hipMemcpyAsync(eq.data(), d_eq, pairs.size() * 4, hipMemcpyDeviceToHost, ctx->stream));
            HIP_TRY(ctx, hipStreamSynchronize(ctx->stream));
            for (size_t k = 0; k < pairs.size(); k++)
                if (eq[k]) {
                    if (rep.empty()) { rep.resize(n); for (uint64_t i = 0; i < n; i++) rep[i] = (uint32_t)i; }
                    rep[pairs[k].x] = pairs[k].y;
                    sp->copies++;
                }
        }
    }
    if (sp->copies) {
        cls_of.assign(n, 0xFFFFFFFFu);
        std::vector<uint32_t> size(n, 0);
        for (uint64_t i = 0; i < n; i++) size[rep[i]]++;
        uint32_t ncls = 0, tot = 0;
        for (uint64_t i = 0; i < n; i++)
            if (size[i] >= 2) { cls_of[i] = ncls++; cls_off.push_back(tot); tot += size[i]; }
        cls_off.push_back(tot);
        cls_rows.resize(tot);
        std::vector<uint32_t> fillp(cls_off.begin(), cls_off.end() - 1);
        for (uint64_t i = 0; i < n; i++) {
            const uint32_t k = cls_of[rep[i]];
            if (k != 0xFFFFFFFFu) cls_rows[fillp[k]++] = (uint32_t)i;
        }
        cls_first.resize(tot);
        for (uint32_t k = 0; k < ncls; k++) {
            const uint64_t m = cls_off[k + 1] - cls_off[k];
            sp->cls_pairs += m * (m - 1) / 2;
            for (uint32_t u = cls_off[k]; u < cls_off[k + 1]; u++) cls_first[u] = cls_off[k];
        }
        sp->cls_members = tot;
        if (ncls == 1 && tot == n && cnt_true[0] > 0) sp->one_class = (uint32_t)cnt_true[0];
        if (sp->one_class && ctx->aside_all_copies) ctx->aside_all_copies(sp->one_class);
    }
    return MG_OK;
}

int SparseIndexBuild::lay_out()
{
    uint64_t E64 = 0;
    sp->off_host.resize(n + 1);
    for (uint64_t i = 0; i < n; i++) {
        sp->off_host[i] = (uint32_t)E64;
        const uint64_t c = cnt_true[i];
        if (rep.empty() || rep[i] == i) E64 += c;
        if (E64 >= (1ull << 31)) return unusable("2^31 entries or more");
        if (c < s) sp->short_rows_host.push_back((uint32_t)i);
        if (c == 0) sp->has_empty = true;
    }
    sp->off_host[n] = (uint32_t)E64;
    if (E64 == 0) return unusable("no hashes");
    E = (uint32_t)E64;
    sp->E = E;
    end_bit = (uint32_t)(64 - __builtin_clzll(maxv | 1ull));
    sort_begin_bit = mg::sparse_sort_begin_bit(E, end_bit, ctx_opt(ctx, "MASHGPU_SPARSE_SORT_BITS"), ctx_opt(ctx, "MASHGPU_SPARSE_SORT_ALL_BITS") != nullptr);
    if (sort_begin_bit > 0 && !ctx_opt(ctx, "MASHGPU_SPARSE_SORT_BITS")) sort_begin_bit = mg::sort_begin_bit_from_density(dens, end_bit, sort_begin_bit);
    lead_lists = mg::dense_sublists();
    lead_cap = std::max<uint32_t>(E / 4u / lead_lists + 64u, 256u);
    if (const char *ev = ctx_opt(ctx, "MASHGPU_DENSE_LEAD_CAP")) lead_cap = std::max<uint32_t>((uint32_t)atoi(ev), 1u);
    const bool tiles_hopeless = ix_tiles && !ix_verify && lab_sorted && !ctx_opt(ctx, "MASHGPU_SPARSE_INDEX") &&
                                longest_label_run(lab_sorted, n) > kTilesLongestRun;
    if (ix_tiles && !tiles_hopeless) plan = mg::index_plan((uint32_t)n, E, s, sp->rs, t->s, maxv, dens0, ix_verify);
    else if (tiles_hopeless) plan.why = "a clade of more rows than a bucket's sort takes";
    if (lb_made && !(plan.ok && memcmp(&plan.g, &early_plan.g, sizeof plan.g) == 0)) lb_made = false;
    temp_bytes = std::max(std::max(mg::sparse_order_temp_bytes((uint32_t)n), mg::sparse_order_slice_temp_bytes((uint32_t)n)),
                          mg::sparse_offsets_temp_bytes((uint32_t)n));
    want_order = !ctx_opt(ctx, "MASHGPU_SPARSE_NO_ORDER");
    ok = temp.alloc(std::max<size_t>(temp_bytes, 16)) == hipSuccess && gs_of.alloc(E) == hipSuccess && d_stat.alloc(1) == hipSuccess &&
              d_slots.alloc(std::max(mg::sparse_stat_scratch_bytes(), mg::index_stat_scratch_bytes())) == hipSuccess &&
              (!want_order || (key64_a.alloc(n) == hipSuccess && key64_b.alloc(n) == hipSuccess));
    ok = ok && take(&sp->off, n + 1) && take(&sp->keys_sorted, E) && take(&sp->gend, E) && take(&sp->sorted_rows, E) &&
         take(&sp->code_img, (size_t)n * sp->rs + 64) && take(&sp->pos_img, (size_t)n * sp->rs) && take(&sp->counters, 4) &&
         (!want_order || take(&sp->order, n));
    nshort = sp->short_rows_host.size();
    short_cnt.assign(nshort, 0);
    for (size_t k = 0; k < nshort; k++) short_cnt[k] = cnt_true[sp->short_rows_host[k]];
    if (ok && nshort) ok = take(&sp->short_rows, nshort) && take(&sp->short_cnt, nshort);
    if (ok && sp->copies)
        ok = take(&sp->rep, n) && take(&sp->cls_of, n) && take(&sp->cls_off, cls_off.size()) && take(&sp->cls_rows, cls_rows.size()) &&
             take(&sp->cls_first, cls_first.size());
    e = hipSuccess;
    if (ok && sp->copies) {
        e = hipMemcpyAsync(sp->rep, rep.data(), n * 4, hipMemcpyHostToDevice, ctx->stream);
        if (e == hipSuccess) e = hipMemcpyAsync(sp->cls_of, cls_of.data(), n * 4, hipMemcpyHostToDevice, ctx->stream);
        if (e == hipSuccess) e = hipMemcpyAsync(sp->cls_off, cls_off.data(), cls_off.size() * 4, hipMemcpyHostToDevice, ctx->stream);
        if (e == hipSuccess) e = hipMemcpyAsync(sp->cls_rows, cls_rows.data(), cls_rows.size() * 4, hipMemcpyHostToDevice, ctx->stream);
        if (e == hipSuccess) e = hipMemcpyAsync(sp->cls_first, cls_first.data(), cls_first.size() * 4, hipMemcpyHostToDevice, ctx->stream);
    }
    if (ok && e == hipSuccess) {
        if (rep.empty()) e = mg::launch_sparse_offsets(d_cnt, cnt_stale ? sp->inv : nullptr, (uint32_t)n, temp, sp->off, ctx->stream);
        else e = hipMemcpyAsync(sp->off, sp->off_host.data(), (n + 1) * 4, hipMemcpyHostToDevice, ctx->stream);
        if (e == hipSuccess && nshort) e = hipMemcpyAsync(sp->short_rows, sp->short_rows_host.data(), nshort * 4, hipMemcpyHostToDevice, ctx->stream);
        if (e == hipSuccess && nshort) e = hipMemcpyAsync(sp->short_cnt, short_cnt.data(), nshort * 4, hipMemcpyHostToDevice, ctx->stream);
    }
    return MG_OK;
}

void SparseIndexBuild::prepare_candidates()
{
    if (cand_prepared) return;
    cand_prepared = true;
    if (link.empty() || sp->copies != 0) return;
    for (uint64_t i = 1; i < n;) {
        if (!link[i]) { i++; continue; }
        uint64_t j = i;
        while (j < n && link[j]) j++;
        if (j - (i - 1) >= 8) {
            mg::DenseGroup g{};
            g.g0 = (uint32_t)(i - 1); g.g1 = (uint32_t)j;
            cand_groups.push_back(g);
        }
        i = j + 1;
    }
    if (cand_groups.empty()) return;
    const uint32_t ng = (uint32_t)cand_groups.size();
    grp_of_h.assign(n, 0xFFFFFFFFu);
    for (uint32_t g = 0; g < ng; g++)
        for (uint32_t r = cand_groups[g].g0; r < cand_groups[g].g1; r++) grp_of_h[r] = g;
    const uint64_t room = (uint64_t)lead_lists * lead_cap;
    if (d_groups.alloc(ng) == hipSuccess && d_grp_of.alloc(n) == hipSuccess && d_lead_rows.alloc(4 * n) == hipSuccess && d_nlead.alloc(2) == hipSuccess && d_cnt_sub.alloc(lead_lists) == hipSuccess &&
        d_off_sub.alloc(lead_lists) == hipSuccess && d_key.alloc(room) == hipSuccess && d_val.alloc(room) == hipSuccess && d_keyj.alloc(room) == hipSuccess &&
        d_valj.alloc(room) == hipSuccess &&
        hipMemcpyAsync(d_groups, cand_groups.data(), ng * sizeof(mg::DenseGroup), hipMemcpyHostToDevice, ctx->stream) == hipSuccess &&
        mg::launch_dense_group_rows(d_groups, ng, (uint32_t)n, d_grp_of, d_lead_rows, ctx->stream) == hipSuccess &&
        hipMemsetAsync(d_cnt_sub, 0, lead_lists * 4, ctx->stream) == hipSuccess && hipMemsetAsync(d_nlead, 0, 8, ctx->stream) == hipSuccess) {
        lead_ready = true;
    } else {
        (void)hipGetLastError();
        cand_groups.clear();
    }
}

void SparseIndexBuild::finish_build()
{
    if (e == hipSuccess && want_order)
        e = mg::launch_sparse_row_order(sp->off, sp->code_img, sp->gend, sp->rep, (uint32_t)n, sp->rs, temp, temp_bytes, key64_a, key64_b,
                                        sp->order, ctx->stream);
    if (e == hipSuccess) e = hipMemcpyAsync(&h_stat, d_stat, sizeof(Stat), hipMemcpyDeviceToHost, ctx->stream);
    if (e == hipSuccess) e = hipStreamSynchronize(ctx->stream);
}

int SparseIndexBuild::build_by_tiles()
{
    if (ok && e == hipSuccess && plan.ok) {
        DevBuf<unsigned char> d_tcnt(ctx), d_start(ctx), d_big(ctx), d_pk(ctx), d_tc(ctx);
        if ((lb_made || d_lb.alloc(plan.lb_bytes) == hipSuccess) && d_tcnt.alloc(plan.cnt_bytes) == hipSuccess && d_start.alloc(plan.start_bytes) == hipSuccess &&
            d_big.alloc(plan.big_bytes) == hipSuccess && d_pk.alloc(plan.pk_bytes) == hipSuccess && d_tc.alloc(plan.tc_bytes) == hipSuccess) {
            e = hipMemsetAsync(d_stat, 0, sizeof(Stat), ctx->stream);
            if (e == hipSuccess)
                e = mg::index_build(plan, H, sp->off, d_lb, d_tcnt, d_start, d_big, d_pk, d_tc, sp->keys_sorted, sp->sorted_rows, sp->gend, gs_of, sp->code_img,
                                    sp->pos_img, d_slots, &d_stat.p->shared, &d_stat.p->max_group, &d_stat.p->groups, d_stat.p->ixf, nullptr, ctx->stream,
                                    lb_made ? 1 | 8 : 1);
            DevBuf<uint32_t> d_swapped(ctx);
            if (e == hipSuccess && ctx_opt(ctx, "MASHGPU_IX_DEBUG_SWAP") && d_swapped.alloc(1) == hipSuccess) {
                e = hipMemsetAsync(d_swapped, 0, 4, ctx->stream);
                if (e == hipSuccess) e = mg::index_debug_swap(plan, d_pk, d_start, d_swapped, ctx->stream);
            }
            prepare_candidates();
            mg::IxLeaders lead;
            if (lead_ready) {
                lead.grp_of = d_lead_rows;
                lead.key = d_key;
                lead.val = d_val;
                lead.cnt = d_cnt_sub;
                lead.cap_sub = lead_cap;
                lead.nsub = lead_lists;
            }
            if (e == hipSuccess && ctx->aside_at_sort) ctx->aside_at_sort();
            if (e == hipSuccess)
                e = mg::index_build(plan, H, sp->off, d_lb, d_tcnt, d_start, d_big, d_pk, d_tc, sp->keys_sorted, sp->sorted_rows, sp->gend, gs_of, sp->code_img,
                                    sp->pos_img, d_slots, &d_stat.p->shared, &d_stat.p->max_group, &d_stat.p->groups, d_stat.p->ixf,
                                    lead_ready ? &lead : nullptr, ctx->stream, 2);
            if (e == hipSuccess && lead_ready) {
                e = mg::dense_join_leaders(d_key, d_val, lead_cap, d_keyj, d_valj, d_cnt_sub, d_off_sub, d_nlead, ctx->stream);
                if (e == hipSuccess) e = hipMemcpyAsync(lead_tot, d_nlead, 8, hipMemcpyDeviceToHost, ctx->stream);
            }
            hipEvent_t ev_stats = nullptr;
            if (e == hipSuccess) e = hipMemcpyAsync(&h_stat, d_stat, sizeof(Stat), hipMemcpyDeviceToHost, ctx->stream);
            if (e == hipSuccess) e = hipEventCreateWithFlags(&ev_stats, hipEventDisableTiming);
            if (e == hipSuccess) e = hipEventRecord(ev_stats, ctx->stream);
            if (e == hipSuccess)
                e = mg::index_build(plan, H, sp->off, d_lb, d_tcnt, d_start, d_big, d_pk, d_tc, sp->keys_sorted, sp->sorted_rows, sp->gend, gs_of, sp->code_img,
                                    sp->pos_img, d_slots, &d_stat.p->shared, &d_stat.p->max_group, &d_stat.p->groups, d_stat.p->ixf,
                                    lead_ready ? &lead : nullptr, ctx->stream, 4);
            if (e == hipSuccess && want_order)
                e = mg::launch_sparse_row_order(sp->off, sp->code_img, sp->gend, sp->rep, (uint32_t)n, sp->rs, temp, temp_bytes, key64_a, key64_b,
                                                sp->order, ctx->stream);
            if (ev_stats) {
                const hipError_t ew = e == hipSuccess ? hipEventSynchronize(ev_stats) : hipStreamSynchronize(ctx->stream);
                if (e == hipSuccess) e = ew;
                (void)hipEventDestroy(ev_stats);
            } else {
                (void)hipStreamSynchronize(ctx->stream);
            }
            built = e == hipSuccess && !h_stat.ixf[mg::IXF_DEGENERATE];
            if (built && lead_ready && lead_tot[1] > lead_cap && h_stat.ixf[mg::IXF_NBIG] == 0) {
                e = hipStreamSynchronize(ctx->stream);
                const uint32_t want_cap = lead_tot[1];
                for (void **q : {(void **)&d_key.p, (void **)&d_val.p, (void **)&d_keyj.p, (void **)&d_valj.p})
                    if (*q) { ctx_free(ctx, *q); *q = nullptr; }
                const uint64_t room = (uint64_t)lead_lists * want_cap;
                if (e == hipSuccess && d_key.alloc(room) == hipSuccess && d_val.alloc(room) == hipSuccess && d_keyj.alloc(room) == hipSuccess &&
                    d_valj.alloc(room) == hipSuccess) {
                    lead_cap = want_cap;
                    lead.key = d_key;
                    lead.val = d_val;
                    lead.cap_sub = lead_cap;
                    e = hipMemsetAsync(d_cnt_sub, 0, lead_lists * 4, ctx->stream);
                    if (e == hipSuccess) e = hipMemsetAsync(d_nlead, 0, 8, ctx->stream);
                    if (e == hipSuccess) e = hipMemsetAsync(d_stat.p, 0, offsetof(Stat, bad), ctx->stream);
                    if (e == hipSuccess)
                        e = mg::index_build(plan, H, sp->off, d_lb, d_tcnt, d_start, d_big, d_pk, d_tc, sp->keys_sorted, sp->sorted_rows, sp->gend, gs_of,
                                            sp->code_img, sp->pos_img, d_slots, &d_stat.p->shared, &d_stat.p->max_group, &d_stat.p->groups, d_stat.p->ixf, &lead,
                                            ctx->stream, 2);
                    if (e == hipSuccess) e = mg::dense_join_leaders(d_key, d_val, lead_cap, d_keyj, d_valj, d_cnt_sub, d_off_sub, d_nlead, ctx->stream);
                    if (e == hipSuccess) e = hipMemcpyAsync(lead_tot, d_nlead, 8, hipMemcpyDeviceToHost, ctx->stream);
                    if (e == hipSuccess) e = hipMemcpyAsync(&h_stat, d_stat, sizeof(Stat), hipMemcpyDeviceToHost, ctx->stream);
                    if (e == hipSuccess) e = hipStreamSynchronize(ctx->stream);
                    built = e == hipSuccess && !h_stat.ixf[mg::IXF_DEGENERATE];
                    if (ctx_opt(ctx, "MASHGPU_SPARSE_DBG"))
                        fprintf(stderr, "compare dense: a list of leaders asked for %u entries: found again with that room (%u leaders)\n", want_cap, lead_tot[0]);
                } else {
                    (void)hipGetLastError();
                }
            }
            lead_done = built && lead_ready;
            if (ctx_opt(ctx, "MASHGPU_SPARSE_DBG"))
                fprintf(stderr, "compare sparse: index by tiles: shift %u, %u buckets (%u per window, %u windows), fullest %u, %u beyond the LDS (%u values streamed)%s\n",
                        plan.g.shift, plan.g.Bp, plan.g.BW, plan.g.NW, h_stat.ixf[mg::IXF_MAXBUCKET], h_stat.ixf[mg::IXF_NBIG], h_stat.ixf[mg::IXF_NSTREAMED],
                        h_stat.ixf[mg::IXF_DEGENERATE] ? " -- clumped values: sorted instead" : "");
        } else {
            (void)hipGetLastError();
        }
    } else if (ix_tiles && ctx_opt(ctx, "MASHGPU_SPARSE_DBG")) {
        fprintf(stderr, "compare sparse: index by tiles refused: %s\n", plan.why);
    }
    sp->by_tiles = built;
    prepare_candidates();
#ifdef IX_PHASE_CLOCKS
    if (built && ctx_opt(ctx, "MASHGPU_IX_CLOCKS")) mg::index_dump_clocks();
#endif
    if (ix_verify && !built && ok && e == hipSuccess && !ctx_opt(ctx, "MASHGPU_SPARSE_INDEX_MAY_REFUSE"))
        return fail(ctx, MG_ERR_INVALID, std::string("index verify: the tile build refused this table (") + (plan.ok ? "bucket flags" : plan.why) + ")");
    return MG_OK;
}

int SparseIndexBuild::build_by_sort()
{
    if (ok && e == hipSuccess && (!built || ix_verify)) {
        const size_t sort_bytes = mg::sparse_sort_temp_bytes(E, end_bit, sort_begin_bit);
        DevBuf<unsigned char> temp_sort(ctx), d_ties(ctx);
        DevBuf<uint64_t> keys_a(ctx), v_keys(ctx);
        DevBuf<uint32_t> idx_a(ctx), idx_sorted(ctx), v_rows(ctx), v_gend(ctx), v_gs(ctx), v_code(ctx), v_pos(ctx);
        DevBuf<unsigned long long> d_diff(ctx);
        bool ok2 = temp_sort.alloc(std::max<size_t>(sort_bytes, 16)) == hipSuccess && keys_a.alloc(E) == hipSuccess && idx_a.alloc(E) == hipSuccess &&
                   idx_sorted.alloc(E) == hipSuccess && d_ties.alloc(mg::sparse_tie_scratch_bytes()) == hipSuccess;
        if (ok2 && built)
            ok2 = v_keys.alloc(E) == hipSuccess && v_rows.alloc(E) == hipSuccess && v_gend.alloc(E) == hipSuccess && v_gs.alloc(E) == hipSuccess &&
                  v_code.alloc((size_t)n * sp->rs + 64) == hipSuccess && v_pos.alloc((size_t)n * sp->rs) == hipSuccess && d_diff.alloc(16) == hipSuccess;
        if (!ok2) {
            (void)hipGetLastError();
            ok = false;
        } else {
            const Stat tiles_stat = h_stat;
            uint64_t *o_keys = built ? v_keys.p : sp->keys_sorted;
            uint32_t *o_rows = built ? v_rows.p : sp->sorted_rows, *o_gend = built ? v_gend.p : sp->gend, *o_gs = built ? v_gs.p : gs_of.p,
                     *o_code = built ? v_code.p : sp->code_img, *o_pos = built ? v_pos.p : sp->pos_img;
            for (uint32_t begin_bit = sort_begin_bit;; begin_bit = 0) {
                if (e == hipSuccess) e = hipMemsetAsync(d_stat, 0, sizeof(Stat), ctx->stream);
                if (e == hipSuccess)
                    e = mg::sparse_build_index(H, t->s, sp->off, (uint32_t)n, E, sp->rs, end_bit, temp_sort, sort_bytes, keys_a, idx_a, o_keys, idx_sorted,
                                               idx_a, o_gs, o_rows, o_gend, o_code, o_pos, d_slots, begin_bit, d_ties, &d_stat.p->shared,
                                               &d_stat.p->max_group, &d_stat.p->groups, &d_stat.p->bad, &d_stat.p->tie_overflow, ctx->stream);
                if (built) {
                    if (e == hipSuccess) e = hipMemcpyAsync(&h_stat, d_stat, sizeof(Stat), hipMemcpyDeviceToHost, ctx->stream);
                    if (e == hipSuccess) e = hipStreamSynchronize(ctx->stream);
                } else {
                    finish_build();
                }
                if (e != hipSuccess || (!h_stat.tie_overflow && !h_stat.bad) || begin_bit == 0) break;
                if (ctx_opt(ctx, "MASHGPU_SPARSE_DBG"))
                    fprintf(stderr, "compare sparse: sort on bits [%u, %u) %s: every bit again\n", begin_bit, end_bit,
                            h_stat.bad ? "left values out of order" : "left ties the repair could not take");
            }
            if (built && e == hipSuccess) {
                unsigned long long diff[16];
                for (int k = 0; k < 8; k++) { diff[2 * k] = 0; diff[2 * k + 1] = ~0ull; }
                e = hipMemcpyAsync(d_diff, diff, sizeof diff, hipMemcpyHostToDevice, ctx->stream);
                const uint64_t img = (uint64_t)n * sp->rs;
                if (e == hipSuccess) e = mg::index_verify_words((const uint32_t *)sp->keys_sorted, (const uint32_t *)v_keys.p, nullptr, 0, 2ull * E, d_diff.p + 0, ctx->stream);
                if (e == hipSuccess) e = mg::index_verify_words(sp->sorted_rows, v_rows, nullptr, 0, E, d_diff.p + 2, ctx->stream);
                if (e == hipSuccess) e = mg::index_verify_words(gs_of, v_gs, nullptr, 0, E, d_diff.p + 4, ctx->stream);
                if (e == hipSuccess) e = mg::index_verify_words(sp->gend, v_gend, v_gs, 1, E, d_diff.p + 6, ctx->stream);
                if (e == hipSuccess) e = mg::index_verify_words(sp->code_img, v_code, nullptr, 0, img, d_diff.p + 8, ctx->stream);
                if (e == hipSuccess) e = mg::index_verify_words(sp->pos_img, v_pos, v_code, 2, img, d_diff.p + 10, ctx->stream);
                if (e == hipSuccess) e = hipMemcpyAsync(diff, d_diff, sizeof diff, hipMemcpyDeviceToHost, ctx->stream);
                if (e == hipSuccess) e = hipStreamSynchronize(ctx->stream);
                if (e == hipSuccess) {
                    static const char *names[6] = {"values (32-bit words)", "rows", "group starts", "group ends", "code image", "position image"};
                    std::string msg;
                    for (int k = 0; k < 6; k++)
                        if (diff[2 * k]) msg += std::string(msg.empty() ? "" : "; ") + names[k] + ": " + std::to_string(diff[2 * k]) + " differ, first at " + std::to_string(diff[2 * k + 1]);
                    if (h_stat.shared != tiles_stat.shared || h_stat.max_group != tiles_stat.max_group || h_stat.groups != tiles_stat.groups)
                        msg += std::string(msg.empty() ? "" : "; ") + "statistics: shared " + std::to_string(tiles_stat.shared) + " / " + std::to_string(h_stat.shared) +
                               ", largest group " + std::to_string(tiles_stat.max_group) + " / " + std::to_string(h_stat.max_group) + ", groups " +
                               std::to_string(tiles_stat.groups) + " / " + std::to_string(h_stat.groups);
                    if (!msg.empty()) {
                        char geom[160];
                        snprintf(geom, sizeof geom, " [n %llu, E %u, shift %u, %u buckets, %u per window, %u windows]", (unsigned long long)n, E, plan.g.shift, plan.g.Bp, plan.g.BW, plan.g.NW);
                        sp->usable = false;
                        return fail(ctx, MG_ERR_INVALID, "index verify: tiles / sort -- " + msg + geom);
                    }
                }
            }
        }
    }
    return MG_OK;
}

int SparseIndexBuild::check_build()
{
    if (!ok) { (void)hipGetLastError(); drop(); return unusable("no device memory for the index"); }
    if (e != hipSuccess) { drop(); return fail(ctx, MG_ERR_HIP, std::string("compare (index build): ") + hipGetErrorString(e)); }
    if (h_stat.bad) { drop(); return unusable("sort order inside a value not by row"); }
    sp->G = h_stat.groups;
    sp->shared = h_stat.shared;
    sp->max_group = h_stat.max_group;
    sp->build_ms = std::chrono::duration<double, std::milli>(std::chrono::steady_clock::now() - t_begin).count();
    sp->usable = true;
    return MG_OK;
}

int SparseIndexBuild::dense_groups()
{
    if (!cand_groups.empty()) {
        auto t_dense = std::chrono::steady_clock::now();
        while (!cand_groups.empty()) {
            const uint32_t ng = (uint32_t)cand_groups.size();
            std::vector<uint32_t> &grp_of = grp_of_h;
            DevBuf<uint32_t> d_us(ctx), d_ue(ctx);
            DevBuf<unsigned long long> d_key2(ctx);
            DevBuf<unsigned char> d_tmp(ctx);
            if (d_us.alloc(ng) != hipSuccess || d_ue.alloc(ng) != hipSuccess) { (void)hipGetLastError(); break; }
            const uint32_t L = lead_lists;
            uint32_t *tot = lead_tot, cap_sub = lead_cap;
            hipError_t e2 = hipSuccess;
            if (!lead_done) {
                if (built || !lead_ready) break;
                for (int attempt = 0; e2 == hipSuccess; attempt++) {
                    if (attempt > 0) {
                        for (void **q : {(void **)&d_key.p, (void **)&d_val.p, (void **)&d_keyj.p, (void **)&d_valj.p})
                            if (*q) { ctx_free(ctx, *q); *q = nullptr; }
                        const uint64_t room = (uint64_t)L * cap_sub;
                        if (d_key.alloc(room) != hipSuccess || d_val.alloc(room) != hipSuccess || d_keyj.alloc(room) != hipSuccess || d_valj.alloc(room) != hipSuccess) {
                            (void)hipGetLastError();
                            e2 = hipErrorOutOfMemory;
                            break;
                        }
                    }
                    e2 = mg::dense_find_leaders(sp->sorted_rows, gs_of, sp->gend, d_grp_of, d_groups, E, d_key, d_val, cap_sub, d_keyj, d_valj, d_cnt_sub, d_off_sub,
                                                d_nlead, ctx->stream);
                    if (e2 == hipSuccess) e2 = hipMemcpyAsync(tot, d_nlead, 8, hipMemcpyDeviceToHost, ctx->stream);
                    if (e2 == hipSuccess) e2 = hipStreamSynchronize(ctx->stream);
                    if (e2 != hipSuccess || tot[1] <= cap_sub || attempt >= 1) break;
                    cap_sub = tot[1];
                }
            } else if (tot[1] > cap_sub && ctx_opt(ctx, "MASHGPU_SPARSE_DBG")) {
                fprintf(stderr, "compare dense: a list of leaders asked for %u entries, room for %u: no dense groups for this table\n", tot[1], cap_sub);
            }
            const uint32_t nlead = tot[0];
            if (e2 != hipSuccess || nlead == 0 || tot[1] > cap_sub) { (void)hipGetLastError(); break; }
            uint32_t gbits = 1;
            while ((1u << gbits) < ng) gbits++;
            std::vector<uint32_t> us(ng, 0), ue(ng, 0);
            void *ul = nullptr, *up = nullptr;
            const size_t tb = mg::dense_universe_temp_bytes(nlead);
            if (d_key2.alloc(nlead) != hipSuccess || d_tmp.alloc(std::max<size_t>(tb, 16)) != hipSuccess ||
                ctx_malloc(ctx, &ul, (size_t)nlead * 4) != hipSuccess || ctx_malloc(ctx, &up, (size_t)nlead * 4) != hipSuccess) {
                (void)hipGetLastError();
                ctx_free(ctx, ul);
                break;
            }
            sp->ulist = static_cast<uint32_t *>(ul);
            sp->upos = static_cast<uint32_t *>(up);
            e2 = hipMemsetAsync(d_us, 0, ng * 4, ctx->stream);
            if (e2 == hipSuccess) e2 = hipMemsetAsync(d_ue, 0, ng * 4, ctx->stream);
            if (e2 == hipSuccess)
                e2 = mg::dense_sort_universes(d_keyj, d_valj, nlead, d_tmp, tb, d_key2, sp->ulist, sp->upos, d_us, d_ue, gbits, ctx->stream);
            if (e2 == hipSuccess) e2 = hipMemcpyAsync(us.data(), d_us, ng * 4, hipMemcpyDeviceToHost, ctx->stream);
            if (e2 == hipSuccess) e2 = hipMemcpyAsync(ue.data(), d_ue, ng * 4, hipMemcpyDeviceToHost, ctx->stream);
            if (e2 == hipSuccess) e2 = hipStreamSynchronize(ctx->stream);
            if (e2 != hipSuccess) { (void)hipGetLastError(); break; }
            const uint32_t kMaxWords = mg::dense_max_words();
            std::fill(grp_of.begin(), grp_of.end(), 0xFFFFFFFFu);
            uint32_t xrows = 0, wmax = 0;
            uint64_t words = 0;
            for (uint32_t g = 0; g < ng; g++) {
                mg::DenseGroup G = cand_groups[g];
                G.u = ue[g] > us[g] ? ue[g] - us[g] : 0u;
                G.ustart = us[g];
                G.W = (G.u >> 6) + 1u;
                if (G.u < 32u || G.W > kMaxWords) continue;
                G.xrow0 = xrows;
                G.data_off = words;
                const uint64_t m = G.g1 - G.g0;
                xrows += (uint32_t)m;
                words += ((m + 127) / 128) * mg::dense_block_words(G.W);
                wmax = std::max(wmax, G.W);
                for (uint32_t r = G.g0; r < G.g1; r++) grp_of[r] = (uint32_t)sp->dgroups_host.size();
                sp->dgroups_host.push_back(G);
            }
            if (sp->dgroups_host.empty()) break;
            sp->dn_wmax = wmax;
            sp->dn_xs = ((s + 7u) & ~7u) + 8u;
            void *p1 = nullptr, *p2 = nullptr, *p3 = nullptr, *p4 = nullptr;
            if (ctx_malloc(ctx, &p1, sp->dgroups_host.size() * sizeof(mg::DenseGroup)) != hipSuccess || ctx_malloc(ctx, &p2, n * 4) != hipSuccess ||
                ctx_malloc(ctx, &p3, words * 8) != hipSuccess || ctx_malloc(ctx, &p4, (size_t)xrows * sp->dn_xs * 2) != hipSuccess) {
                (void)hipGetLastError();
                for (void *q : {p1, p2, p3, p4}) ctx_free(ctx, q);
                sp->dgroups_host.clear();
                break;
            }
            sp->dgroups = static_cast<mg::DenseGroup *>(p1);
            sp->grp_of = static_cast<uint32_t *>(p2);
            sp->gdata = static_cast<unsigned long long *>(p3);
            sp->ext = static_cast<uint16_t *>(p4);
            e2 = hipMemcpyAsync(sp->dgroups, sp->dgroups_host.data(), sp->dgroups_host.size() * sizeof(mg::DenseGroup), hipMemcpyHostToDevice, ctx->stream);
            if (e2 == hipSuccess) e2 = hipMemcpyAsync(sp->grp_of, grp_of.data(), n * 4, hipMemcpyHostToDevice, ctx->stream);
            if (e2 == hipSuccess)
                e2 = mg::launch_dense_encode(sp->off, sp->code_img, sp->pos_img, sp->rs, sp->grp_of, sp->dgroups, sp->ulist, sp->upos, sp->gdata,
                                             sp->ext, sp->dn_xs, (uint32_t)n, wmax, ctx->stream,
                                             ctx_opt(ctx, "MASHGPU_DENSE_UL_LDS") ? atoi(ctx_opt(ctx, "MASHGPU_DENSE_UL_LDS")) : -1);
            sp->grp_of_host.swap(grp_of);
            if (e2 != hipSuccess) {
                drop();
                for (void **q : {(void **)&sp->dgroups, (void **)&sp->grp_of, (void **)&sp->gdata, (void **)&sp->ext, (void **)&sp->ulist,
                                 (void **)&sp->upos})
                    if (*q) { ctx_free(ctx, *q); *q = nullptr; }
                sp->dgroups_host.clear();
                sp->usable = false;
                return fail(ctx, MG_ERR_HIP, std::string("compare (index build, dense groups): ") + hipGetErrorString(e2));
            }
            sp->dn_lists = ctx_opt(ctx, "MASHGPU_DENSE_LISTS") != nullptr;
            break;
        }
        if (sp->dgroups_host.empty() && sp->ulist) { ctx_free(ctx, sp->ulist); ctx_free(ctx, sp->upos); sp->ulist = sp->upos = nullptr; }
        sp->build_ms += std::chrono::duration<double, std::milli>(std::chrono::steady_clock::now() - t_dense).count();
        if (ctx_opt(ctx, "MASHGPU_SPARSE_DBG")) {
            uint64_t rows_in = 0;
            for (auto &G : sp->dgroups_host) rows_in += G.g1 - G.g0;
            fprintf(stderr, "compare dense: %zu chains of related rows, %zu groups kept (%llu rows, widest universe %u words)\n", cand_groups.size(),
                    sp->dgroups_host.size(), (unsigned long long)rows_in, sp->dn_wmax);
        }
    }
    if (ctx_opt(ctx, "MASHGPU_SPARSE_DBG"))
        fprintf(stderr, "compare sparse: index of %llu rows (%llu copies of earlier rows), s %u: %u entries, %u distinct, shared %llu, largest run %u, %.2f ms\n",
                (unsigned long long)n, (unsigned long long)sp->copies, s, E, sp->G, (unsigned long long)sp->shared, sp->max_group, sp->build_ms);
    return MG_OK;
}

int SparseIndexBuild::run()
{
    int rc = MG_OK;
    if ((rc = scan_rows()) != MG_OK || stop) return rc;
    if ((rc = order_rows()) != MG_OK || stop) return rc;
    if ((rc = find_copies()) != MG_OK || stop) return rc;
    if ((rc = lay_out()) != MG_OK || stop) return rc;
    if ((rc = build_by_tiles()) != MG_OK || stop) return rc;
    if ((rc = build_by_sort()) != MG_OK || stop) return rc;
    if ((rc = check_build()) != MG_OK || stop) return rc;
    return dense_groups();
}

}

int table_sparse_index(mg_ctx *ctx, const mg_table *t, uint32_t s, bool clustered, mg_table::Sparse **out, uint32_t split)
{
    if (!clustered) split = 0;
    for (mg_table::Sparse *sp : t->sparse)
        if (sp->s == s && sp->clustered == clustered && sp->split == split) { *out = sp; return MG_OK; }
    mg_table::Sparse *sp = new mg_table::Sparse;
    sp->s = s;
    sp->clustered = clustered;
    sp->split = split;
    t->sparse.push_back(sp);
    *out = sp;
    auto unusable = [&](const char *why) { sp->usable = false; sp->why = why; return MG_OK; };
    const uint64_t n = t->n;
    if (n == 0) return unusable("empty table");
// ... 10 lines not shown
```

### mash_amd/csrc/mashgpu.cpp

```cpp
#include "host_internal.h"

namespace {

thread_local std::string g_create_error;

std::mutex g_live_mu;
std::vector<const void *> g_live_ctx;

}

bool ctx_is_live(const void *c)
{
    std::lock_guard<std::mutex> lk(g_live_mu);
    return std::find(g_live_ctx.begin(), g_live_ctx.end(), c) != g_live_ctx.end();
}

void ctx_trim(mg_ctx *ctx)
{
    for (auto &b : ctx->blk_free) hipFree(b.p);
    ctx->blk_free.clear();
    ctx->blk_cached = 0;
    for (auto &b : ctx->big_free) hipFree(b.p);
    ctx->big_free.clear();
    ctx->big_cached = 0;
// ... 65 lines not shown
            ctx->big_cached += b.bytes;
        } else {
            hipFree(p);
        }
        return;
    }
    hipFree(p);
}

int fail(mg_ctx *ctx, int code, const std::string &msg)
{
    if (ctx) ctx->err = msg; else g_create_error = msg;
    return code;
}

void *ctx_pinned(mg_ctx *ctx, size_t bytes)
{
    if (bytes <= ctx->pin_cap) return ctx->pin;
    if (ctx->pin) (void)hipHostFree(ctx->pin);
    ctx->pin = nullptr;
    ctx->pin_cap = 0;
    const size_t cap = bytes + bytes / 4 + 4096;
    if (hipHostMalloc(&ctx->pin, cap, hipHostMallocDefault) != hipSuccess) {
        (void)hipGetLastError();
        ctx->pin = nullptr;
        return nullptr;
    }
    ctx->pin_cap = cap;
    return ctx->pin;
}

const char *ctx_opt(const mg_ctx *ctx, const char *name)
{
    if (ctx) {
        const auto it = ctx->options.find(name);
        if (it != ctx->options.end()) return it->second.c_str();
    }
    return getenv(name);
}

void prof_begin(mg_ctx *ctx, std::vector<ProfRec> &v, hipStream_t stream)
{
    if (!ctx->prof) return;
    ProfRec r;
    hipEventCreate(&r.a);
    hipEventCreate(&r.b);
    hipEventRecord(r.a, stream ? stream : ctx->stream);
    v.push_back(r);
}

void prof_end(mg_ctx *ctx, std::vector<ProfRec> &v, hipStream_t stream)
{
    if (!ctx->prof || v.empty()) return;
    hipEventRecord(v.back().b, stream ? stream : ctx->stream);
}


int mg_device_count(void)
{
    int n = 0;
    if (hipGetDeviceCount(&n) != hipSuccess) { (void)hipGetLastError(); return 0; }
    return n;
}

int mg_ctx_create(int device, mg_ctx **out)
{
    if (!out) return fail(nullptr, MG_ERR_INVALID, "mg_ctx_create: out is NULL");
    int ndev = 0;
    hipError_t e = hipGetDeviceCount(&ndev);
    if (e != hipSuccess || ndev == 0)
        return fail(nullptr, MG_ERR_HIP, std::string("no HIP device: ") + hipGetErrorString(e));
    if (device < 0 || device >= ndev) return fail(nullptr, MG_ERR_INVALID, "mg_ctx_create: bad device index");
    e = hipSetDevice(device);
    if (e != hipSuccess) return fail(nullptr, MG_ERR_HIP, std::string("hipSetDevice: ") + hipGetErrorString(e));
    mg_ctx *c = new mg_ctx;
    c->device = device;
    e = hipStreamCreateWithFlags(&c->stream, hipStreamDefault);
    if (e != hipSuccess) { delete c; return fail(nullptr, MG_ERR_HIP, "hipStreamCreate failed"); }
    c->own_stream = true;
    int cus = 0;
    if (hipDeviceGetAttribute(&cus, hipDeviceAttributeMultiprocessorCount, device) == hipSuccess) c->cu_count = cus;
    {
        size_t free_b = 0, total_b = 0;
        if (hipMemGetInfo(&free_b, &total_b) == hipSuccess && total_b) c->big_limit = std::max<size_t>(c->big_limit, total_b / 10 * 4);
        else (void)hipGetLastError();
    }
    { std::lock_guard<std::mutex> lk(g_live_mu); g_live_ctx.push_back(c); }
    *out = c;
    return MG_OK;
}

void mg_ctx_destroy(mg_ctx *ctx)
{
    if (!ctx) return;
    { std::lock_guard<std::mutex> lk(g_live_mu); g_live_ctx.erase(std::remove(g_live_ctx.begin(), g_live_ctx.end(), (const void *)ctx), g_live_ctx.end()); }
    mg_prof_reset(ctx);
    for (auto &c : ctx->cost_clk) { if (c.a) hipEventDestroy(c.a); if (c.b) hipEventDestroy(c.b); }
    for (auto &sl : ctx->slots) {
        if (sl.dev) hipFree(sl.dev);
        if (sl.host) hipHostFree(sl.host);
        if (sl.done) hipEventDestroy(sl.done);
    }
    ctx_trim(ctx);
    for (auto &b : ctx->blk_live) hipFree(b.p);
    if (ctx->pin) hipHostFree(ctx->pin);
    if (ctx->aux) { hipStreamDestroy(ctx->aux); hipEventDestroy(ctx->aux_go); hipEventDestroy(ctx->aux_done); hipFree(ctx->aux_ctr); ctx->aux = nullptr; }
    if (ctx->own_stream && ctx->stream) hipStreamDestroy(ctx->stream);
    delete ctx;
}

const char *mg_last_error(mg_ctx *ctx) { return ctx ? ctx->err.c_str() : g_create_error.c_str(); }

int mg_ctx_trim(mg_ctx *ctx)
{
    if (!ctx) return MG_ERR_INVALID;
    std::lock_guard<std::recursive_mutex> lk(ctx->mu);
    HIP_TRY(ctx, hipSetDevice(ctx->device));
    HIP_TRY(ctx, hipStreamSynchronize(ctx->stream));
    ctx_trim(ctx);
    return MG_OK;
}

int mg_ctx_set_stream(mg_ctx *ctx, void *hip_stream)
{
    if (!ctx) return MG_ERR_INVALID;
    std::lock_guard<std::recursive_mutex> lk(ctx->mu);
    if (ctx->own_stream && ctx->stream) { hipStreamDestroy(ctx->stream); ctx->own_stream = false; }
    if (hip_stream == nullptr) {
        HIP_TRY(ctx, hipStreamCreateWithFlags(&ctx->stream, hipStreamDefault));
        ctx->own_stream = true;
    } else {
        ctx->stream = (hipStream_t)hip_stream;
    }
    return MG_OK;
}

int mg_ctx_set_option(mg_ctx *ctx, const char *name, const char *value)
{
    if (!ctx) return MG_ERR_INVALID;
    std::lock_guard<std::recursive_mutex> lk(ctx->mu);
    if (!name || strncmp(name, "MASHGPU_", 8) != 0) return fail(ctx, MG_ERR_INVALID, "mg_ctx_set_option: knob names start with MASHGPU_");
    if (value) ctx->options[name] = value; else ctx->options.erase(name);
    return MG_OK;
}

int mg_ctx_set_async(mg_ctx *ctx, int on)
{
    if (!ctx) return MG_ERR_INVALID;
    std::lock_guard<std::recursive_mutex> lk(ctx->mu);
    ctx->async = on != 0;
    return MG_OK;
}

int mg_ctx_synchronize(mg_ctx *ctx)
{
    if (!ctx) return MG_ERR_INVALID;
    std::lock_guard<std::recursive_mutex> lk(ctx->mu);
    HIP_TRY(ctx, hipSetDevice(ctx->device));
    HIP_TRY(ctx, hipStreamSynchronize(ctx->stream));
    return MG_OK;
}

int mg_ctx_cu_count(mg_ctx *ctx) { return ctx ? ctx->cu_count : 0; }

int mg_params_init(mg_params *p, int kmer_size, uint64_t sketch_size, uint32_t seed,
                   const char *alphabet, int noncanonical, int preserve_case)
{
    if (!p || !alphabet || kmer_size < 1 || kmer_size > 32 || sketch_size < 1) return MG_ERR_INVALID;
    memset(p, 0, sizeof *p);
    p->kmer_size = kmer_size;
    p->sketch_size = sketch_size;
    p->seed = seed;
    p->noncanonical = noncanonical ? 1 : 0;
    p->preserve_case = preserve_case ? 1 : 0;
    p->min_copies = 1;
    p->target_cov = 0.0;
    p->bloom_bytes = 0;
    for (const char *c = alphabet; *c; c++) {
        char u = *c;
        if (!preserve_case && u > 96 && u < 123) u -= 32;
        p->alphabet[(unsigned char)u] = 1;
    }
    for (int i = 0; i < 256; i++) p->alphabet_size += p->alphabet[i] ? 1 : 0;
    p->use64 = pow((double)p->alphabet_size, (double)kmer_size) > pow(2.0, 32.0);
    return MG_OK;
}


int mg_table_upload(mg_ctx *ctx, const uint64_t *hashes, const uint32_t *nhash, const uint64_t *lengths,
                    uint64_t n, uint64_t s, mg_table **out)
{
    if (!ctx) return MG_ERR_INVALID;
    std::lock_guard<std::recursive_mutex> lk(ctx->mu);
    if (!hashes || !nhash || !out || s == 0) return fail(ctx, MG_ERR_INVALID, "mg_table_upload: bad argument");
    HIP_TRY(ctx, hipSetDevice(ctx->device));
    DevBuf<uint64_t> dh(ctx), dl(ctx);
    DevBuf<uint32_t> dn(ctx);
    if (dh.alloc(n * s) != hipSuccess || dn.alloc(n) != hipSuccess || dl.alloc(n) != hipSuccess)
        return fail(ctx, MG_ERR_NOMEM, "mg_table_upload: device allocation failed");
    HIP_TRY(ctx, hipMemcpyAsync(dh, hashes, n * s * 8, hipMemcpyHostToDevice, ctx->stream));
    HIP_TRY(ctx, hipMemcpyAsync(dn, nhash, n * 4, hipMemcpyHostToDevice, ctx->stream));
    if (lengths) HIP_TRY(ctx, hipMemcpyAsync(dl, lengths, n * 8, hipMemcpyHostToDevice, ctx->stream));
    else HIP_TRY(ctx, hipMemsetAsync(dl, 0, n * 8, ctx->stream));
    HIP_TRY(ctx, hipStreamSynchronize(ctx->stream));
    mg_table *t = new mg_table;
    t->ctx = ctx; t->hashes = dh.release(); t->nhash = dn.release(); t->lengths = dl.release(); t->n = n; t->s = s; t->owns = true;
    *out = t;
    return MG_OK;
}

int mg_table_wrap_dev(mg_ctx *ctx, const uint64_t *hashes_dev, const uint32_t *nhash_dev,
                      const uint64_t *lengths_dev, uint64_t n, uint64_t s, mg_table **out)
{
    if (!ctx) return MG_ERR_INVALID;
    std::lock_guard<std::recursive_mutex> lk(ctx->mu);
    if (!hashes_dev || !nhash_dev || !out || s == 0) return fail(ctx, MG_ERR_INVALID, "mg_table_wrap_dev: bad argument");
    mg_table *t = new mg_table;
    t->ctx = ctx; t->hashes = hashes_dev; t->nhash = nhash_dev; t->lengths = lengths_dev;
    t->n = n; t->s = s; t->owns = false;
    *out = t;
    return MG_OK;
}

static void table_drop_derived(mg_table *t)
{
    mg_ctx *ctx = t->ctx;
    for (mg_table *v : t->prefix_views) { table_drop_derived(v); delete v; }
    t->prefix_views.clear();
    if (!t->pfx.empty() || !t->win.empty() || !t->sparse.empty()) hipSetDevice(ctx->device);
    for (auto &im : t->pfx) ctx_free(ctx, im.second);
    t->pfx.clear();
    for (auto &w : t->win) ctx_free(ctx, w.dev);
    t->win.clear();
    for (mg_table::Sparse *sp : t->sparse) {
        for (auto &pl : sp->plans) {
            if (pl.order) ctx_free(ctx, pl.order);
            if (pl.dtiles) ctx_free(ctx, pl.dtiles);
        }
        for (void *q : {(void *)sp->off, (void *)sp->keys_sorted, (void *)sp->gend, (void *)sp->sorted_rows,
                        (void *)sp->pos_img, (void *)sp->code_img, (void *)sp->short_rows, (void *)sp->short_cnt, (void *)sp->cand,
                        (void *)sp->res, (void *)sp->seg_base, (void *)sp->seg_cnt, (void *)sp->chunks, (void *)sp->chunk_inc,
                        sp->scan_temp, (void *)sp->counters, (void *)sp->rep, (void *)sp->cls_of, (void *)sp->cls_off,
                        (void *)sp->cls_rows, (void *)sp->cls_first, (void *)sp->order, (void *)sp->dgroups, (void *)sp->grp_of,
                        (void *)sp->ulist, (void *)sp->upos, (void *)sp->gdata, (void *)sp->ext, (void *)sp->inv, (void *)sp->phashes})
            if (q) ctx_free(ctx, q);
        for (void *q : sp->jn.bufs)
            if (q) ctx_free(ctx, q);
        delete sp;
    }
    t->sparse.clear();
    t->cls.clear();
    t->last.clear();
    t->nh.clear();
    t->have_max = false;
}

const mg_table *table_prefix_view(const mg_table *t, uint64_t n)
{
    if (n >= t->n) return t;
    for (mg_table *v : t->prefix_views)
        if (v->n == n) return v;
    if (t->prefix_views.size() >= 4) {
        table_drop_derived(t->prefix_views.front());
        delete t->prefix_views.front();
        t->prefix_views.erase(t->prefix_views.begin());
    }
    mg_table *v = new mg_table;
    v->ctx = t->ctx;
    v->hashes = t->hashes;
    v->nhash = t->nhash;
    v->lengths = t->lengths;
    v->n = n;
    v->s = t->s;
    v->owns = false;
    t->prefix_views.push_back(v);
    return v;
}

void mg_table_free(mg_table *t)
{
    if (!t) return;
    if (!ctx_is_live(t->ctx)) { delete t; return; }
    {
        std::lock_guard<std::recursive_mutex> lk(t->ctx->mu);
        table_drop_derived(t);
        if (t->owns) {
            hipSetDevice(t->ctx->device);
            ctx_free(t->ctx, (void *)t->hashes);
            ctx_free(t->ctx, (void *)t->nhash);
            ctx_free(t->ctx, (void *)t->lengths);
        }
    }
    delete t;
}

int mg_table_invalidate(mg_table *t)
{
    if (!t || !ctx_is_live(t->ctx)) return MG_ERR_INVALID;
    std::lock_guard<std::recursive_mutex> lk(t->ctx->mu);
    table_drop_derived(t);
    return MG_OK;
}

uint64_t mg_table_rows(const mg_table *t) { return t ? t->n : 0; }
uint64_t mg_table_sketch_size(const mg_table *t) { return t ? t->s : 0; }


int mg_prof_enable(mg_ctx *ctx, int on)
{
    if (!ctx) return MG_ERR_INVALID;
    std::lock_guard<std::recursive_mutex> lk(ctx->mu);
    ctx->prof = on != 0;
    return MG_OK;
}

void mg_prof_reset(mg_ctx *ctx)
{
    if (!ctx) return;
    for (auto *v : {&ctx->prof_compare, &ctx->prof_sketch, &ctx->prof_fill, &ctx->prof_discover, &ctx->prof_merge, &ctx->prof_index, &ctx->prof_dense, &ctx->prof_join, &ctx->prof_fill_aside}) {
        for (auto &r : *v) { hipEventDestroy(r.a); hipEventDestroy(r.b); }
        v->clear();
    }
}

double mg_prof_avg_ms(mg_ctx *ctx, const char *name, uint64_t *launches_out)
{
    if (launches_out) *launches_out = 0;
    if (!ctx || !name) return 0.0;
    std::vector<ProfRec> *v = nullptr;
    if (strcmp(name, "compare") == 0) v = &ctx->prof_compare;
    else if (strcmp(name, "sketch") == 0) v = &ctx->prof_sketch;
    else if (strcmp(name, "compare_fill") == 0) v = &ctx->prof_fill;
    else if (strcmp(name, "compare_fill_aside") == 0) v = &ctx->prof_fill_aside;
    else if (strcmp(name, "compare_discover") == 0) v = &ctx->prof_discover;
    else if (strcmp(name, "compare_merge") == 0) v = &ctx->prof_merge;
    else if (strcmp(name, "compare_index") == 0) v = &ctx->prof_index;
    else if (strcmp(name, "compare_dense") == 0) v = &ctx->prof_dense;
    else if (strcmp(name, "compare_join") == 0) v = &ctx->prof_join;
    if (!v || v->empty()) return 0.0;
    hipStreamSynchronize(ctx->stream);
    double tot = 0.0;
    uint64_t n = 0;
    for (auto &r : *v) {
        float ms = 0.f;
        if (hipEventElapsedTime(&ms, r.a, r.b) == hipSuccess) { tot += ms; n++; }
    }
    if (launches_out) *launches_out = n;
    return n ? tot / (double)n : 0.0;
}
```

Before: 429.5 billion pairs/s.

## Replace sort-based row clustering and dedup prescan with GPU hash tables

Clustering by first hashes now inserts each row's first four hashes into an open-addressed hash table and keeps the minimum row per hash, instead of doing a 64-bit radix sort of 4n pairs followed by binary searches. The final ordering sort uses 32-bit keys with only the needed label bits and a counting iterator for values. The duplicate-digest prescan now uses a hash probe that is initialised inside the digest kernel, and the full sort-based suspect detection plus its buffers are deferred until a duplicate is actually flagged. Row-order keys are narrowed as well. The aim is to cut index-build overhead per step. The cost is atomic contention on the tables and a fixed number of label jumps that may not fully converge.

```diff
diff --git a/mash_amd/csrc/compare_dense.hip b/mash_amd/csrc/compare_dense.hip
--- a/mash_amd/csrc/compare_dense.hip
+++ b/mash_amd/csrc/compare_dense.hip
@@ -625,85 +625,126 @@
 #ifndef MG_HIP_EMU
 constexpr uint32_t CL_FIRST = 4;
 
-__global__ __launch_bounds__(256) void cl_emit_kernel(const uint64_t *hashes, uint64_t stride, const uint32_t *cnt, uint32_t n,
-                                                      unsigned long long *key, uint32_t *row_out, uint32_t *label)
+static uint32_t cl_slots(uint32_t n)
+{
+    uint32_t slots = 16;
+    while (slots < 2ull * CL_FIRST * n) slots <<= 1;
+    return slots;
+}
+
+static uint32_t cl_label_bits(uint32_t n) { return n > 1 ? 32u - (uint32_t)__builtin_clz(n - 1u) : 1u; }
+
+__device__ inline uint32_t cl_home(uint64_t h, uint32_t mask)
+{
+    h = (h ^ (h >> 30)) * 0xBF58476D1CE4E5B9ull;
+    h = (h ^ (h >> 27)) * 0x94D049BB133111EBull;
+    return (uint32_t)(h ^ (h >> 31)) & mask;
+}
+
+__device__ inline uint32_t cl_find(unsigned long long *tkey, uint32_t mask, unsigned long long h, bool insert)
+{
+    uint32_t slot = cl_home(h, mask);
+    for (uint32_t step = 0; step <= mask; step++) {
+        const unsigned long long k = insert ? atomicCAS(&tkey[slot], ~0ull, h) : tkey[slot];
+        if (k == h || (insert && k == ~0ull)) return slot;
+        slot = (slot + 1u) & mask;
+    }
+    return 0xFFFFFFFFu;
+}
+
+__global__ __launch_bounds__(256) void cl_insert_kernel(const uint64_t *hashes, uint64_t stride, const uint32_t *cnt, uint32_t n,
+                                                        unsigned long long *tkey, uint32_t *tmin, uint32_t mask)
 {
     const uint32_t i = blockIdx.x * 256u + threadIdx.x;
     if (i >= n * CL_FIRST) return;
     const uint32_t row = i / CL_FIRST, f = i % CL_FIRST;
-    key[i] = f < cnt[row] ? (unsigned long long)hashes[(uint64_t)row * stride + f] : ~0ull;
-    row_out[i] = row;
-    if (f == 0) label[row] = row;
-}
-
-__global__ __launch_bounds__(256) void cl_minrow_kernel(const unsigned long long *key_sorted, const uint32_t *row_sorted, uint32_t m,
-                                                        uint32_t *label)
-{
+    if (f >= cnt[row]) return;
+    const unsigned long long h = hashes[(uint64_t)row * stride + f];
+    if (h == ~0ull) return;
+    const uint32_t slot = cl_find(tkey, mask, h, true);
+    if (slot != 0xFFFFFFFFu) atomicMin(&tmin[slot], row);
+}
+
+__global__ __launch_bounds__(256) void cl_label_kernel(const uint64_t *hashes, uint64_t stride, const uint32_t *cnt, uint32_t n,
+                                                       unsigned long long *tkey, const uint32_t *tmin, uint32_t mask, uint32_t *label)
+{
+    static_assert(CL_FIRST == 4, "four lanes a row");
     const uint32_t i = blockIdx.x * 256u + threadIdx.x;
-    if (i >= m) return;
-    const unsigned long long k = key_sorted[i];
-    if (k == ~0ull) return;
-    uint32_t lo = 0, hi = i;
-    while (lo < hi) {
-        const uint32_t mid = (lo + hi) >> 1;
-        if (key_sorted[mid] < k) lo = mid + 1; else hi = mid;
-    }
-    atomicMin(&label[row_sorted[i]], row_sorted[lo]);
-}
-
-__global__ __launch_bounds__(256) void cl_jump_kernel(const uint32_t *in, uint32_t *out, uint32_t n)
+    const uint32_t row = i / CL_FIRST, f = i % CL_FIRST;
+    uint32_t v = row;
+    if (row < n && f < cnt[row]) {
+        const unsigned long long h = hashes[(uint64_t)row * stride + f];
+        if (h != ~0ull) {
+            const uint32_t slot = cl_find(tkey, mask, h, false);
+            if (slot != 0xFFFFFFFFu) v = min(v, tmin[slot]);
+        }
+    }
+    v = min(v, (uint32_t)__shfl_xor((int)v, 1));
+    v = min(v, (uint32_t)__shfl_xor((int)v, 2));
+    if (row < n && f == 0) label[row] = v;
+}
+
+__global__ __launch_bounds__(256) void cl_order_keys_kernel(const uint32_t *label, uint32_t n, uint32_t split, uint32_t lbits, uint32_t *key)
 {
     const uint32_t i = blockIdx.x * 256u + threadIdx.x;
-    if (i < n) out[i] = in[in[i]];
-}
-
-__global__ __launch_bounds__(256) void cl_order_keys_kernel(const uint32_t *label, uint32_t n, uint32_t split, unsigned long long *key)
+    if (i < n) key[i] = ((i >= split ? 1u : 0u) << lbits) | label[label[label[label[i]]]];
+}
+
+__global__ __launch_bounds__(256) void cl_labels_sorted_kernel(const uint32_t *key_sorted, uint32_t n, uint32_t lmask, uint32_t *label_sorted)
 {
     const uint32_t i = blockIdx.x * 256u + threadIdx.x;
-    if (i < n) key[i] = ((unsigned long long)(i >= split ? 1u : 0u) << 63) | ((unsigned long long)label[i] << 32) | i;
-}
-
-__global__ __launch_bounds__(256) void cl_split_keys_kernel(const unsigned long long *key_sorted, uint32_t n, uint32_t *inv, uint32_t *label_sorted)
-{
-    const uint32_t i = blockIdx.x * 256u + threadIdx.x;
-    if (i < n) {
-        inv[i] = (uint32_t)(key_sorted[i] & 0xFFFFFFFFull);
-        label_sorted[i] = (uint32_t)(key_sorted[i] >> 32) & 0x7FFFFFFFu;
-    }
-}
-
-size_t dense_cluster_temp_bytes(uint32_t n)
-{
-    size_t a = 0, b = 0;
-    rocprim::radix_sort_pairs(nullptr, a, (const unsigned long long *)nullptr, (unsigned long long *)nullptr, (const uint32_t *)nullptr,
-                              (uint32_t *)nullptr, (size_t)n * CL_FIRST, 0u, 64u, (hipStream_t) nullptr);
-    rocprim::radix_sort_keys(nullptr, b, (const unsigned long long *)nullptr, (unsigned long long *)nullptr, (size_t)n, 0u, 64u,
-                             (hipStream_t) nullptr);
-    return a > b ? a : b;
-}
+    if (i < n) label_sorted[i] = key_sorted[i] & lmask;
+}
+
+struct ClScratch {
+    unsigned long long *tkey;
+    uint32_t *tmin, *key_a, *key_b;
+    void *sort_temp;
+    size_t sort_bytes, table_bytes, total;
+};
+
+static ClScratch cl_scratch(uint32_t n, void *base)
+{
+    ClScratch c;
+    const uint32_t slots = cl_slots(n);
+    const size_t npad = ((size_t)n + 63u) & ~(size_t)63u;
+    c.sort_bytes = 0;
+    rocprim::radix_sort_pairs(nullptr, c.sort_bytes, (const uint32_t *)nullptr, (uint32_t *)nullptr, rocprim::counting_iterator<uint32_t>(0u),
+                              (uint32_t *)nullptr, (size_t)n, 0u, cl_label_bits(n) + 1u, (hipStream_t) nullptr);
+    unsigned char *p = static_cast<unsigned char *>(base);
+    c.table_bytes = ((size_t)slots * 12u + 255u) & ~(size_t)255u;
+    c.tkey = reinterpret_cast<unsigned long long *>(p);
+    c.tmin = reinterpret_cast<uint32_t *>(p + (size_t)slots * 8u);
+    c.key_a = reinterpret_cast<uint32_t *>(p + c.table_bytes);
+    c.key_b = c.key_a + npad;
+    c.sort_temp = p + c.table_bytes + 8u * npad;
+    c.total = c.table_bytes + 8u * npad + c.sort_bytes;
+    return c;
+}
+
+size_t dense_cluster_temp_bytes(uint32_t n) { return cl_scratch(n, nullptr).total; }
 
 hipError_t dense_cluster_rows(const uint64_t *hashes, uint64_t stride, const uint32_t *cnt, uint32_t n, void *temp, size_t temp_bytes,
-                              unsigned long long *key_a, unsigned long long *key_b, uint32_t *row_a, uint32_t *row_b, uint32_t *lab_a,
-                              uint32_t *lab_b, uint32_t *inv, uint32_t *label_sorted, hipStream_t stream, uint32_t split)
+                              uint32_t *lab, uint32_t *inv, uint32_t *label_sorted, hipStream_t stream, uint32_t split)
 {
     if (n == 0) return hipSuccess;
-    const uint32_t m = n * CL_FIRST;
-    hipLaunchKernelGGL(cl_emit_kernel, dim3((m + 255u) / 256u), dim3(256), 0, stream, hashes, stride, cnt, n, key_a, row_a, lab_a);
-    hipError_t e = hipGetLastError();
+    const ClScratch c = cl_scratch(n, temp);
+    if (temp_bytes < c.total) return hipErrorInvalidValue;
+    const uint32_t m = n * CL_FIRST, mask = cl_slots(n) - 1u, lbits = cl_label_bits(n);
+    hipError_t e = hipMemsetAsync(c.tkey, 0xFF, (size_t)(mask + 1u) * 12u, stream);
     if (e != hipSuccess) return e;
-    e = rocprim::radix_sort_pairs(temp, temp_bytes, (const unsigned long long *)key_a, key_b, (const uint32_t *)row_a, row_b, (size_t)m, 0u, 64u,
-                                  stream);
-    if (e != hipSuccess) return e;
-    hipLaunchKernelGGL(cl_minrow_kernel, dim3((m + 255u) / 256u), dim3(256), 0, stream, (const unsigned long long *)key_b, (const uint32_t *)row_b, m,
-                       lab_a);
-    hipLaunchKernelGGL(cl_jump_kernel, dim3((n + 255u) / 256u), dim3(256), 0, stream, (const uint32_t *)lab_a, lab_b, n);
-    hipLaunchKernelGGL(cl_jump_kernel, dim3((n + 255u) / 256u), dim3(256), 0, stream, (const uint32_t *)lab_b, lab_a, n);
-    hipLaunchKernelGGL(cl_order_keys_kernel, dim3((n + 255u) / 256u), dim3(256), 0, stream, (const uint32_t *)lab_a, n, split, key_a);
+    hipLaunchKernelGGL(cl_insert_kernel, dim3((m + 255u) / 256u), dim3(256), 0, stream, hashes, stride, cnt, n, c.tkey, c.tmin, mask);
+    hipLaunchKernelGGL(cl_label_kernel, dim3((m + 255u) / 256u), dim3(256), 0, stream, hashes, stride, cnt, n, c.tkey, (const uint32_t *)c.tmin,
+                       mask, lab);
+    hipLaunchKernelGGL(cl_order_keys_kernel, dim3((n + 255u) / 256u), dim3(256), 0, stream, (const uint32_t *)lab, n, split, lbits, c.key_a);
     e = hipGetLastError();
     if (e != hipSuccess) return e;
-    e = rocprim::radix_sort_keys(temp, temp_bytes, (const unsigned long long *)key_a, key_b, (size_t)n, 0u, 64u, stream);
+    size_t sort_bytes = c.sort_bytes;
+    e = rocprim::radix_sort_pairs(c.sort_temp, sort_bytes, (const uint32_t *)c.key_a, c.key_b, rocprim::counting_iterator<uint32_t>(0u), inv,
+                                  (size_t)n, 0u, lbits + 1u, stream);
     if (e != hipSuccess) return e;
-    hipLaunchKernelGGL(cl_split_keys_kernel, dim3((n + 255u) / 256u), dim3(256), 0, stream, (const unsigned long long *)key_b, n, inv, label_sorted);
+    hipLaunchKernelGGL(cl_labels_sorted_kernel, dim3((n + 255u) / 256u), dim3(256), 0, stream, (const uint32_t *)c.key_b, n,
+                       (uint32_t)((1ull << lbits) - 1u), label_sorted);
     return hipGetLastError();
 }
 
diff --git a/mash_amd/csrc/compare_internal.h b/mash_amd/csrc/compare_internal.h
--- a/mash_amd/csrc/compare_internal.h
+++ b/mash_amd/csrc/compare_internal.h
@@ -97,12 +97,15 @@
     const DenseGroup *dn_groups;
 };
 size_t sparse_dup_temp_bytes(uint32_t n);
+uint32_t sparse_dup_probe_words(uint32_t n);
+hipError_t launch_sparse_dup_probe(const unsigned long long *dig, const uint32_t *cnt, uint32_t n, unsigned long long *probe, uint32_t *nflag,
+                                   hipStream_t stream);
 hipError_t launch_sparse_dup_suspects(const unsigned long long *dig, const uint32_t *cnt, uint32_t n, void *temp, size_t temp_bytes,
                                       unsigned long long *dig_sorted, uint32_t *rows_sorted, uint32_t *flags, uint32_t *nflag,
                                       hipStream_t stream);
-size_t sparse_order_temp_bytes(uint32_t n);
+size_t sparse_order_temp_bytes(uint32_t n, uint32_t E);
 hipError_t launch_sparse_row_order(const uint32_t *off, const uint32_t *code_img, const uint32_t *gend, const uint32_t *rep, uint32_t n,
-                                   uint32_t rs, void *temp, size_t temp_bytes, unsigned long long *key_a, unsigned long long *key_b,
+                                   uint32_t rs, uint32_t E, void *temp, size_t temp_bytes, unsigned long long *key_a, unsigned long long *key_b,
                                    uint32_t *order, hipStream_t stream);
 size_t sparse_order_slice_temp_bytes(uint32_t n);
 hipError_t launch_sparse_order_slice(const uint32_t *order, uint32_t n, uint32_t rb, uint32_t re, void *temp, size_t temp_bytes,
@@ -111,7 +114,7 @@
                                      const uint32_t *rep, uint32_t members, uint32_t row_begin, uint32_t row_end, uint64_t out_base,
                                      const uint32_t *inv, hipStream_t stream);
 hipError_t launch_sparse_row_digest(const uint64_t *hashes, uint64_t stride, const uint32_t *cnt, uint32_t n,
-                                    unsigned long long *digest, hipStream_t stream);
+                                    unsigned long long *digest, hipStream_t stream, unsigned long long *probe = nullptr, uint32_t *nflag = nullptr);
 hipError_t launch_sparse_row_equal(const uint64_t *hashes, uint64_t stride, const uint32_t *cnt, const uint2 *pairs, uint32_t npairs,
                                    uint32_t *equal, hipStream_t stream);
 hipError_t launch_sparse_row_counts(const uint32_t *nhash, uint32_t n, uint32_t cap, uint32_t *cnt, hipStream_t stream);
@@ -205,8 +208,7 @@
                               hipStream_t stream, const DenseList *list = nullptr);
 size_t dense_cluster_temp_bytes(uint32_t n);
 hipError_t dense_cluster_rows(const uint64_t *hashes, uint64_t stride, const uint32_t *cnt, uint32_t n, void *temp, size_t temp_bytes,
-                              unsigned long long *key_a, unsigned long long *key_b, uint32_t *row_a, uint32_t *row_b, uint32_t *lab_a,
-                              uint32_t *lab_b, uint32_t *inv, uint32_t *label_sorted, hipStream_t stream, uint32_t split = 0);
+                              uint32_t *lab, uint32_t *inv, uint32_t *label_sorted, hipStream_t stream, uint32_t split = 0);
 hipError_t launch_dense_gather_rows(const uint64_t *hashes, uint64_t stride, const uint32_t *inv, uint32_t n, uint64_t *out, hipStream_t stream);
 hipError_t launch_dense_group_rows(const DenseGroup *groups, uint32_t ng, uint32_t n, uint32_t *grp_of, uint32_t *lead_rows, hipStream_t stream);
 
diff --git a/mash_amd/csrc/compare_sparse.hip b/mash_amd/csrc/compare_sparse.hip
--- a/mash_amd/csrc/compare_sparse.hip
+++ b/mash_amd/csrc/compare_sparse.hip
@@ -179,9 +179,14 @@
 
 
 __global__ __launch_bounds__(256) void sp_row_digest_kernel(const uint64_t *hashes, uint64_t stride, const uint32_t *cnt,
-                                                            unsigned long long *digest)
+                                                            unsigned long long *digest, unsigned long long *probe, uint32_t probe_words,
+                                                            uint32_t *nflag)
 {
     const uint32_t row = blockIdx.x;
+    if (probe) {
+        if (threadIdx.x < 4u && 4u * row + threadIdx.x < probe_words) probe[4u * row + threadIdx.x] = ~0ull;
+        if (row == 0 && threadIdx.x == 0) *nflag = 0;
+    }
     const uint32_t n = cnt[row];
     const uint64_t *src = hashes + (uint64_t)row * stride;
     unsigned long long h = 0;
@@ -213,10 +218,11 @@
 }
 
 hipError_t launch_sparse_row_digest(const uint64_t *hashes, uint64_t stride, const uint32_t *cnt, uint32_t n,
-                                    unsigned long long *digest, hipStream_t stream)
+                                    unsigned long long *digest, hipStream_t stream, unsigned long long *probe, uint32_t *nflag)
 {
     if (n == 0) return hipSuccess;
-    hipLaunchKernelGGL(sp_row_digest_kernel, dim3(n), dim3(256), 0, stream, hashes, stride, cnt, digest);
+    hipLaunchKernelGGL(sp_row_digest_kernel, dim3(n), dim3(256), 0, stream, hashes, stride, cnt, digest, probe,
+                       probe ? sparse_dup_probe_words(n) : 0u, nflag);
     return hipGetLastError();
 }
 
@@ -242,6 +248,51 @@
     if (f) atomicAdd(nflag, 1u);
 }
 
+static uint32_t dup_probe_slots(uint32_t n)
+{
+    uint32_t slots = 2;
+    while (slots < 2ull * n) slots <<= 1;
+    return slots;
+}
+
+uint32_t sparse_dup_probe_words(uint32_t n) { return dup_probe_slots(n) + 1u; }
+
+__device__ inline uint64_t sp_mix64(uint64_t z)
+{
+    z = (z ^ (z >> 30)) * 0xBF58476D1CE4E5B9ull;
+    z = (z ^ (z >> 27)) * 0x94D049BB133111EBull;
+    return z ^ (z >> 31);
+}
+
+__global__ __launch_bounds__(256) void sp_dup_probe_kernel(const unsigned long long *dig, const uint32_t *cnt, uint32_t n,
+                                                           unsigned long long *probe, uint32_t mask, uint32_t *nflag)
+{
+    const uint32_t i = blockIdx.x * 256u + threadIdx.x;
+    if (i >= n || cnt[i] == 0) return;
+    const unsigned long long d = dig[i];
+    bool seen = true;
+    if (d == ~0ull) {
+        seen = atomicCAS(&probe[mask + 1u], ~0ull, 0ull) != ~0ull;
+    } else {
+        uint32_t slot = (uint32_t)sp_mix64(d) & mask;
+        for (uint32_t step = 0; step <= mask; step++) {
+            const unsigned long long prev = atomicCAS(&probe[slot], ~0ull, d);
+            if (prev == ~0ull) { seen = false; break; }
+            if (prev == d) break;
+            slot = (slot + 1u) & mask;
+        }
+    }
+    if (seen) atomicAdd(nflag, 1u);
+}
+
+hipError_t launch_sparse_dup_probe(const unsigned long long *dig, const uint32_t *cnt, uint32_t n, unsigned long long *probe, uint32_t *nflag,
+                                   hipStream_t stream)
+{
+    if (n == 0) return hipSuccess;
+    hipLaunchKernelGGL(sp_dup_probe_kernel, dim3((n + 255u) / 256u), dim3(256), 0, stream, dig, cnt, n, probe, dup_probe_slots(n) - 1u, nflag);
+    return hipGetLastError();
+}
+
 size_t sparse_dup_temp_bytes(uint32_t n)
 {
     size_t b = 0;
@@ -265,13 +316,14 @@
 }
 
 __global__ __launch_bounds__(256) void sp_row_key_kernel(const uint32_t *off, const uint32_t *code_img, const uint32_t *gend,
-                                                         const uint32_t *rep, uint32_t n, uint32_t rs, unsigned long long *key64)
+                                                         const uint32_t *rep, uint32_t n, uint32_t rs, uint32_t none, uint32_t *key,
+                                                         uint32_t *row_of)
 {
     const uint32_t row = blockIdx.x * 4u + (threadIdx.x >> 6), lane = threadIdx.x & 63u;
     if (row >= n) return;
     const uint32_t er = rep ? rep[row] : row;
     const uint32_t cnt = off[er + 1] - off[er];
-    uint32_t k = 0xFFFFFFFFu;
+    uint32_t k = none;
     for (uint32_t base = 0; base < cnt; base += 64u) {
         const uint32_t p = base + lane;
         const uint32_t code = p < cnt ? code_img[(uint64_t)er * rs + p] : 0u;
@@ -281,35 +333,33 @@
             break;
         }
     }
-    if (lane == 0) key64[row] = ((unsigned long long)k << 32) | (unsigned long long)(0xFFFFFFFFu - row);
-}
-
-__global__ __launch_bounds__(256) void sp_order_from_keys_kernel(const unsigned long long *key64_sorted, uint32_t n, uint32_t *order)
-{
-    const uint32_t i = blockIdx.x * 256u + threadIdx.x;
-    if (i < n) order[i] = 0xFFFFFFFFu - (uint32_t)(key64_sorted[i] & 0xFFFFFFFFull);
-}
-
-size_t sparse_order_temp_bytes(uint32_t n)
+    if (lane == 0) {
+        key[n - 1u - row] = k;
+        row_of[n - 1u - row] = row;
+    }
+}
+
+static uint32_t order_key_bits(uint32_t E) { return E ? 32u - (uint32_t)__builtin_clz(E) : 1u; }
+
+size_t sparse_order_temp_bytes(uint32_t n, uint32_t E)
 {
     size_t b = 0;
-    rocprim::radix_sort_keys(nullptr, b, (const unsigned long long *)nullptr, (unsigned long long *)nullptr, (size_t)n, 0u, 64u,
-                             (hipStream_t) nullptr);
+    rocprim::radix_sort_pairs(nullptr, b, (const uint32_t *)nullptr, (uint32_t *)nullptr, (const uint32_t *)nullptr, (uint32_t *)nullptr,
+                              (size_t)n, 0u, order_key_bits(E), (hipStream_t) nullptr);
     return b;
 }
 
 hipError_t launch_sparse_row_order(const uint32_t *off, const uint32_t *code_img, const uint32_t *gend, const uint32_t *rep, uint32_t n,
-                                   uint32_t rs, void *temp, size_t temp_bytes, unsigned long long *key_a, unsigned long long *key_b,
+                                   uint32_t rs, uint32_t E, void *temp, size_t temp_bytes, unsigned long long *key_a, unsigned long long *key_b,
                                    uint32_t *order, hipStream_t stream)
 {
     if (n == 0) return hipSuccess;
-    hipLaunchKernelGGL(sp_row_key_kernel, dim3((n + 3u) / 4u), dim3(256), 0, stream, off, code_img, gend, rep, n, rs, key_a);
+    uint32_t *key_in = reinterpret_cast<uint32_t *>(key_a), *row_in = key_in + n, *key_out = reinterpret_cast<uint32_t *>(key_b);
+    hipLaunchKernelGGL(sp_row_key_kernel, dim3((n + 3u) / 4u), dim3(256), 0, stream, off, code_img, gend, rep, n, rs, E, key_in, row_in);
     hipError_t e = hipGetLastError();
     if (e != hipSuccess) return e;
-    e = rocprim::radix_sort_keys(temp, temp_bytes, (const unsigned long long *)key_a, key_b, (size_t)n, 0u, 64u, stream);
-    if (e != hipSuccess) return e;
-    hipLaunchKernelGGL(sp_order_from_keys_kernel, dim3((n + 255u) / 256u), dim3(256), 0, stream, (const unsigned long long *)key_b, n, order);
-    return hipGetLastError();
+    return rocprim::radix_sort_pairs(temp, temp_bytes, (const uint32_t *)key_in, key_out, (const uint32_t *)row_in, order, (size_t)n, 0u,
+                                     order_key_bits(E), stream);
 }
 
 struct sp_in_range {
diff --git a/mash_amd/csrc/host_index.cpp b/mash_amd/csrc/host_index.cpp
--- a/mash_amd/csrc/host_index.cpp
+++ b/mash_amd/csrc/host_index.cpp
@@ -34,8 +34,8 @@
 
     bool need_classes = false, dedup = true, want_dense = true, try_cluster = false, try_links = false;
     DevBuf<uint8_t> dc_cls, d_link;
-    DevBuf<unsigned long long> dc_last, d_dig, d_dig_sorted, k_a, k_b;
-    DevBuf<uint32_t> d_cnt, d_rows_sorted, d_flags, d_nflag, r_a, r_b, l_a, l_b, d_inv, d_lab;
+    DevBuf<unsigned long long> dc_last, d_dig, d_dig_sorted, d_probe;
+    DevBuf<uint32_t> d_cnt, d_rows_sorted, d_flags, d_nflag, l_a, d_inv, d_lab;
     DevBuf<unsigned char> d_tmp_dup, d_tmp_cl;
     std::vector<uint8_t> hc_cls, link;
     std::vector<uint64_t> hc_last;
@@ -86,7 +86,7 @@
 
     SparseIndexBuild(mg_ctx *c, const mg_table *tab, uint32_t sketch_size, bool clustered_variant, mg_table::Sparse *index, uint32_t split_row)
         : ctx(c), t(tab), s(sketch_size), clustered(clustered_variant), split(split_row), sp(index), n(tab->n), dc_cls(c), d_link(c), dc_last(c), d_dig(c),
-          d_dig_sorted(c), k_a(c), k_b(c), d_cnt(c), d_rows_sorted(c), d_flags(c), d_nflag(c), r_a(c), r_b(c), l_a(c), l_b(c), d_inv(c),
+          d_dig_sorted(c), d_probe(c), d_cnt(c), d_rows_sorted(c), d_flags(c), d_nflag(c), l_a(c), d_inv(c),
           d_lab(c), d_tmp_dup(c), d_tmp_cl(c), d_lb(c), d_groups(c), d_grp_of(c), d_lead_rows(c), d_val(c), d_valj(c), d_cnt_sub(c),
           d_off_sub(c), d_nlead(c), d_key(c), d_keyj(c), temp(c), gs_of(c), key64_a(c), key64_b(c), d_stat(c), d_slots(c)
     {
@@ -144,11 +144,10 @@
     if (const char *v = ctx_opt(ctx, "MASHGPU_COMPARE_DENSE")) want_dense = atoi(v) != 0;
     try_cluster = clustered && n >= 16;
     try_links = !try_cluster && want_dense && n >= 8 && s <= 16384;
-    tb_dup = mg::sparse_dup_temp_bytes((uint32_t)n);
     tb_cl = mg::dense_cluster_temp_bytes((uint32_t)n);
     if (d_cnt.alloc(n) != hipSuccess || (need_classes && (dc_cls.alloc(n) != hipSuccess || dc_last.alloc(n) != hipSuccess)) ||
-        (dedup && (d_dig.alloc(n) != hipSuccess || d_dig_sorted.alloc(n) != hipSuccess || d_rows_sorted.alloc(n) != hipSuccess ||
-                   d_flags.alloc(n) != hipSuccess || d_nflag.alloc(1) != hipSuccess || d_tmp_dup.alloc(std::max<size_t>(tb_dup, 16)) != hipSuccess))) {
+        (dedup && (d_dig.alloc(n) != hipSuccess || d_probe.alloc(mg::sparse_dup_probe_words((uint32_t)n)) != hipSuccess ||
+                   d_nflag.alloc(1) != hipSuccess))) {
         (void)hipGetLastError();
         return unusable("no device memory for the index");
     }
@@ -162,15 +161,13 @@
         }
         if (e == hipSuccess) e = mg::launch_sparse_row_counts(t->nhash, (uint32_t)n, (uint32_t)std::min<uint64_t>(t->s, s), d_cnt, ctx->stream);
         if (e == hipSuccess && dedup) {
-            e = mg::launch_sparse_row_digest(t->hashes, t->s, d_cnt, (uint32_t)n, d_dig, ctx->stream);
-            if (e == hipSuccess)
-                e = mg::launch_sparse_dup_suspects(d_dig, d_cnt, (uint32_t)n, d_tmp_dup, tb_dup, d_dig_sorted, d_rows_sorted, d_flags, d_nflag, ctx->stream);
+            e = mg::launch_sparse_row_digest(t->hashes, t->s, d_cnt, (uint32_t)n, d_dig, ctx->stream, d_probe, d_nflag);
+            if (e == hipSuccess) e = mg::launch_sparse_dup_probe(d_dig, d_cnt, (uint32_t)n, d_probe, d_nflag, ctx->stream);
         }
         if (e == hipSuccess && try_cluster) {
-            if (k_a.alloc(4 * n) == hipSuccess && k_b.alloc(4 * n) == hipSuccess && r_a.alloc(4 * n) == hipSuccess && r_b.alloc(4 * n) == hipSuccess &&
-                l_a.alloc(n) == hipSuccess && l_b.alloc(n) == hipSuccess && d_inv.alloc(n) == hipSuccess && d_lab.alloc(n) == hipSuccess &&
+            if (l_a.alloc(n) == hipSuccess && d_inv.alloc(n) == hipSuccess && d_lab.alloc(n) == hipSuccess &&
                 d_tmp_cl.alloc(std::max<size_t>(tb_cl, 16)) == hipSuccess) {
-                e = mg::dense_cluster_rows(t->hashes, t->s, d_cnt, (uint32_t)n, d_tmp_cl, tb_cl, k_a, k_b, r_a, r_b, l_a, l_b, d_inv, d_lab, ctx->stream, split);
+                e = mg::dense_cluster_rows(t->hashes, t->s, d_cnt, (uint32_t)n, d_tmp_cl, tb_cl, l_a, d_inv, d_lab, ctx->stream, split);
                 cluster_q = true;
             } else {
                 (void)hipGetLastError();
@@ -307,6 +304,12 @@
 int SparseIndexBuild::find_copies()
 {
     if (dedup && nflag) {
+        tb_dup = mg::sparse_dup_temp_bytes((uint32_t)n);
+        if (d_dig_sorted.alloc(n) != hipSuccess || d_rows_sorted.alloc(n) != hipSuccess || d_flags.alloc(n) != hipSuccess ||
+            d_tmp_dup.alloc(std::max<size_t>(tb_dup, 16)) != hipSuccess) {
+            (void)hipGetLastError();
+            return unusable("no device memory for the index");
+        }
         HIP_TRY(ctx, counts_to_device());
         HIP_TRY(ctx, mg::launch_sparse_row_digest(H, t->s, d_cnt, (uint32_t)n, d_dig, ctx->stream));
         HIP_TRY(ctx, mg::launch_sparse_dup_suspects(d_dig, d_cnt, (uint32_t)n, d_tmp_dup, tb_dup, d_dig_sorted, d_rows_sorted, d_flags, d_nflag, ctx->stream));
@@ -393,7 +396,7 @@
     if (ix_tiles && !tiles_hopeless) plan = mg::index_plan((uint32_t)n, E, s, sp->rs, t->s, maxv, dens0, ix_verify);
     else if (tiles_hopeless) plan.why = "a clade of more rows than a bucket's sort takes";
     if (lb_made && !(plan.ok && memcmp(&plan.g, &early_plan.g, sizeof plan.g) == 0)) lb_made = false;
-    temp_bytes = std::max(std::max(mg::sparse_order_temp_bytes((uint32_t)n), mg::sparse_order_slice_temp_bytes((uint32_t)n)),
+    temp_bytes = std::max(std::max(mg::sparse_order_temp_bytes((uint32_t)n, E), mg::sparse_order_slice_temp_bytes((uint32_t)n)),
                           mg::sparse_offsets_temp_bytes((uint32_t)n));
     want_order = !ctx_opt(ctx, "MASHGPU_SPARSE_NO_ORDER");
     ok = temp.alloc(std::max<size_t>(temp_bytes, 16)) == hipSuccess && gs_of.alloc(E) == hipSuccess && d_stat.alloc(1) == hipSuccess &&
@@ -464,7 +467,7 @@
 void SparseIndexBuild::finish_build()
 {
     if (e == hipSuccess && want_order)
-        e = mg::launch_sparse_row_order(sp->off, sp->code_img, sp->gend, sp->rep, (uint32_t)n, sp->rs, temp, temp_bytes, key64_a, key64_b,
+        e = mg::launch_sparse_row_order(sp->off, sp->code_img, sp->gend, sp->rep, (uint32_t)n, sp->rs, E, temp, temp_bytes, key64_a, key64_b,
                                         sp->order, ctx->stream);
     if (e == hipSuccess) e = hipMemcpyAsync(&h_stat, d_stat, sizeof(Stat), hipMemcpyDeviceToHost, ctx->stream);
     if (e == hipSuccess) e = hipStreamSynchronize(ctx->stream);
@@ -514,7 +517,7 @@
                                     sp->pos_img, d_slots, &d_stat.p->shared, &d_stat.p->max_group, &d_stat.p->groups, d_stat.p->ixf,
                                     lead_ready ? &lead : nullptr, ctx->stream, 4);
             if (e == hipSuccess && want_order)
-                e = mg::launch_sparse_row_order(sp->off, sp->code_img, sp->gend, sp->rep, (uint32_t)n, sp->rs, temp, temp_bytes, key64_a, key64_b,
+                e = mg::launch_sparse_row_order(sp->off, sp->code_img, sp->gend, sp->rep, (uint32_t)n, sp->rs, E, temp, temp_bytes, key64_a, key64_b,
                                                 sp->order, ctx->stream);
             if (ev_stats) {
                 const hipError_t ew = e == hipSuccess ? hipEventSynchronize(ev_stats) : hipStreamSynchronize(ctx->stream);
diff --git a/mash_amd/csrc/mashgpu.cpp b/mash_amd/csrc/mashgpu.cpp
--- a/mash_amd/csrc/mashgpu.cpp
+++ b/mash_amd/csrc/mashgpu.cpp
@@ -391,6 +391,32 @@
     return MG_OK;
 }
 
+extern "C" int mg_test_index_prephase(mg_table *t, uint32_t s, uint32_t split, uint32_t *nflag_out, uint32_t *inv_out, uint32_t *label_out)
+{
+    if (!t || !ctx_is_live(t->ctx)) return MG_ERR_INVALID;
+    mg_ctx *ctx = t->ctx;
+    std::lock_guard<std::recursive_mutex> lk(ctx->mu);
+    const uint32_t n = (uint32_t)t->n;
+    DevBuf<uint32_t> cnt(ctx), nflag(ctx), lab(ctx), inv(ctx), lab_sorted(ctx);
+    DevBuf<unsigned long long> dig(ctx), probe(ctx);
+    DevBuf<unsigned char> temp(ctx);
+    const size_t tb = mg::dense_cluster_temp_bytes(n);
+    if (cnt.alloc(n) != hipSuccess || nflag.alloc(1) != hipSuccess || lab.alloc(n) != hipSuccess || inv.alloc(n) != hipSuccess ||
+        lab_sorted.alloc(n) != hipSuccess || dig.alloc(n) != hipSuccess || probe.alloc(mg::sparse_dup_probe_words(n)) != hipSuccess ||
+        temp.alloc(std::max<size_t>(tb, 16)) != hipSuccess)
+        return fail(ctx, MG_ERR_HIP, "test_index_prephase: no device memory");
+    hipError_t e = mg::launch_sparse_row_counts(t->nhash, n, (uint32_t)std::min<uint64_t>(t->s, s), cnt, ctx->stream);
+    if (e == hipSuccess) e = mg::launch_sparse_row_digest(t->hashes, t->s, cnt, n, dig, ctx->stream, probe, nflag);
+    if (e == hipSuccess) e = mg::launch_sparse_dup_probe(dig, cnt, n, probe, nflag, ctx->stream);
+    if (e == hipSuccess) e = mg::dense_cluster_rows(t->hashes, t->s, cnt, n, temp, tb, lab, inv, lab_sorted, ctx->stream, split);
+    if (e == hipSuccess) e = hipMemcpyAsync(nflag_out, nflag, 4, hipMemcpyDeviceToHost, ctx->stream);
+    if (e == hipSuccess) e = hipMemcpyAsync(inv_out, inv, (size_t)n * 4, hipMemcpyDeviceToHost, ctx->stream);
+    if (e == hipSuccess) e = hipMemcpyAsync(label_out, lab_sorted, (size_t)n * 4, hipMemcpyDeviceToHost, ctx->stream);
+    const hipError_t es = hipStreamSynchronize(ctx->stream);
+    if (e == hipSuccess) e = es;
+    return e == hipSuccess ? MG_OK : fail(ctx, MG_ERR_HIP, std::string("test_index_prephase: ") + hipGetErrorString(e));
+}
+
 uint64_t mg_table_rows(const mg_table *t) { return t ? t->n : 0; }
 uint64_t mg_table_sketch_size(const mg_table *t) { return t ? t->s : 0; }
 
```

Result: no change. 432.5 billion pairs/s, median of 6 (+0.7%).
